# hzeller/timg

Measured on NVIDIA H100. Metric: Mpixels/s scale+dither+sixel-encode @4K→cell, higher is better.
Workload: dtype u8/f32

## Files before the change

### timg_b200/csrc/sixel.cu

```cuda
#include <cstdlib>

#include "sixel.cuh"

namespace b200timg {

constexpr int PT = 1024;

__device__ __forceinline__ int pick_plane(int d0, int d1, int d2) {
    const double lum[3] = {0.2989, 0.5866, 0.1145};
    const int spreads[3] = {d0 << 3, d1 << 3, d2 << 3};
    int plane = 0; double best = 0.0;
#pragma unroll
    for (int p = 0; p < 3; ++p) { const double sp = lum[p] * (double)spreads[p]; if (sp > best) { plane = p; best = sp; } }
    return plane;
}

template <bool SMEM_TABLES>
__global__ void __launch_bounds__(PT)
sixel_palette_kernel(const uint32_t *__restrict__ fb, int w, int h, SixelWork W) {
    extern __shared__ uint32_t s_hist[];
    __shared__ uint32_t s_w[PT / 32];
    __shared__ int b_ind[256], b_col[256], b_med[256], t_ind[256], t_col[256], t_med[256];
    __shared__ uint32_t b_sum[256], b_low[256], t_sum[256], t_low[256];
    __shared__ int s_mn[3], s_mx[3];
    __shared__ uint32_t s_cnt[32], s_base[32], s_run[32];
    __shared__ unsigned short s_wh[32][32];
    __shared__ uint32_t w_cnt[32][32], w_base[32][32], w_run[32][32];
    __shared__ int s_todo[32], s_ntodo, s_boxes, s_done;
    __shared__ unsigned long long s_med;

    const int f = blockIdx.x, tid = threadIdx.x, lane = tid & 31, wid = tid >> 5;
    const long long npix = (long long)w * h;
    const uint32_t *frame = fb + (long long)f * npix;
    SixelFrameHdr *hdr = W.hdr + f;
    const int t_words = W.ent_cap > 16384 ? W.ent_cap : 16384;
    uint32_t *E = SMEM_TABLES ? s_hist + t_words : W.ent_a + (long long)f * W.ent_cap;
    uint32_t *T = SMEM_TABLES ? s_hist : W.ent_b + (long long)f * W.ent_cap;

    unsigned long long step_px = (unsigned long long)npix / 18383ull;
    if ((unsigned long long)npix < 18383ull) step_px = 6;
    if (step_px == 0) step_px = 1;
    const long long ns = (npix + (long long)step_px - 1) / (long long)step_px;

    for (int i = tid; i < 16384; i += PT) s_hist[i] = 0;
    __syncthreads();
    for (long long k = tid; k < ns; k += PT) {
        const uint32_t b = hash15(frame[k * (long long)step_px]);
        atomicAdd(&s_hist[b >> 1], 1u << (16 * (b & 1)));
    }
    __syncthreads();
    uint32_t mine = 0;
    for (int k = 0; k < 16; ++k) { const uint32_t v = s_hist[tid * 16 + k]; mine += ((v & 0xffff) != 0) + ((v >> 16) != 0); }
    uint32_t n_ent;
    uint32_t pos = block_excl_scan<PT>(mine, s_w, n_ent);
    for (int k = 0; k < 16; ++k) {
        const uint32_t v = s_hist[tid * 16 + k];
        const uint32_t b0 = (uint32_t)(tid * 32 + 2 * k);
        if (v & 0xffff) E[pos++] = (b0 << 16) | (v & 0xffff);
        if (v >> 16) E[pos++] = ((b0 + 1) << 16) | (v >> 16);
    }
    __syncthreads();
    if (tid == 0) { hdr->origcolors = n_ent; hdr->diffuse = n_ent > 256 ? 1 : 0; }
    if (n_ent <= 256) {
        if (tid < 256) {
            uint32_t pal = 0;
            if ((uint32_t)tid < n_ent) { const uint32_t e = E[tid]; pal = (key5(e, 0) << 3) | (key5(e, 1) << 11) | (key5(e, 2) << 19); }
            hdr->palette[tid] = pal;
        }
        if (tid == 0) hdr->ncolors = n_ent;
        return;
    }
    {
        uint32_t sacc = 0;
        for (uint32_t i = tid; i < n_ent; i += PT) sacc += E[i] & 0xffff;
        uint32_t total; const uint32_t dummy = block_excl_scan<PT>(sacc, s_w, total); (void)dummy;
        if (tid == 0) { b_ind[0] = 0; b_col[0] = (int)n_ent; b_sum[0] = total; b_med[0] = -1; s_boxes = 1; s_done = 0; }
    }
    for (;;) {
        __syncthreads();
        if (wid == 0) {
            const int nb = s_boxes;
            int count = 0;
            for (int c0 = 0; c0 < nb; c0 += 32) {
                const int j = c0 + lane;
                const bool flag = j < nb && b_col[j] >= 2 && b_med[j] < 0;
                const uint32_t m = __ballot_sync(0xffffffffu, flag);
                const int pos = count + __popc(m & ((1u << lane) - 1));
                if (flag && pos < 32) s_todo[pos] = j;
                count += __popc(m);
            }
            if (lane == 0) s_ntodo = min(count, 32);
        }
        __syncthreads();
        const int ntodo = s_ntodo;
        for (int t = 0; t < ntodo; ++t) {
            const int bi = s_todo[t];
            const int start = b_ind[bi], size = b_col[bi];
            if (size <= 1024) continue;
            const uint32_t sm = b_sum[bi];
            uint32_t *B = E + start, *TB = T + start;
            if (tid == 0) { s_mn[0] = s_mn[1] = s_mn[2] = 31; s_mx[0] = s_mx[1] = s_mx[2] = 0; s_med = ~0ull; }
            if (tid < 32) { s_cnt[tid] = 0; s_run[tid] = 0; }
            __syncthreads();
            int mn0 = 31, mn1 = 31, mn2 = 31, mx0 = 0, mx1 = 0, mx2 = 0;
            for (int i = tid; i < size; i += PT) {
                const uint32_t e = B[i];
                const int k0 = key5(e, 0), k1 = key5(e, 1), k2 = key5(e, 2);
                mn0 = min(mn0, k0); mx0 = max(mx0, k0); mn1 = min(mn1, k1); mx1 = max(mx1, k1); mn2 = min(mn2, k2); mx2 = max(mx2, k2);
            }
#pragma unroll
            for (int d = 16; d; d >>= 1) {
                mn0 = min(mn0, __shfl_xor_sync(0xffffffffu, mn0, d)); mx0 = max(mx0, __shfl_xor_sync(0xffffffffu, mx0, d));
                mn1 = min(mn1, __shfl_xor_sync(0xffffffffu, mn1, d)); mx1 = max(mx1, __shfl_xor_sync(0xffffffffu, mx1, d));
                mn2 = min(mn2, __shfl_xor_sync(0xffffffffu, mn2, d)); mx2 = max(mx2, __shfl_xor_sync(0xffffffffu, mx2, d));
            }
            if (lane == 0) {
                atomicMin(&s_mn[0], mn0); atomicMax(&s_mx[0], mx0); atomicMin(&s_mn[1], mn1); atomicMax(&s_mx[1], mx1);
                atomicMin(&s_mn[2], mn2); atomicMax(&s_mx[2], mx2);
            }
            __syncthreads();
            const int plane = pick_plane(s_mx[0] - s_mn[0], s_mx[1] - s_mn[1], s_mx[2] - s_mn[2]);
            for (int i = tid; i < size; i += PT) atomicAdd(&s_cnt[key5(B[i], plane)], 1u);
            __syncthreads();
            if (tid < 32) {
                const uint32_t c = s_cnt[tid]; uint32_t inc = c;
#pragma unroll
                for (int d = 1; d < 32; d <<= 1) { const uint32_t o = __shfl_up_sync(0xffffffffu, inc, d); if (lane >= d) inc += o; }
                s_base[tid] = inc - c;
            }
            for (int t0 = 0; t0 < size; t0 += PT) {
                s_wh[wid][lane] = 0;
                __syncthreads();
                const int i = t0 + tid;
                const bool valid = i < size;
                uint32_t e = 0, k = 0, rank = 0;
                const uint32_t vmask = __ballot_sync(0xffffffffu, valid);
                if (valid) {
                    e = B[i]; k = key5(e, plane);
                    const uint32_t m = __match_any_sync(vmask, k);
                    rank = __popc(m & ((1u << lane) - 1));
                    if (rank == 0) s_wh[wid][k] = (unsigned short)__popc(m);
                }
                __syncthreads();
                if (valid) {
                    uint32_t pp = s_base[k] + s_run[k] + rank;
                    for (int w2 = 0; w2 < wid; ++w2) pp += s_wh[w2][k];
                    TB[pp] = e;
                }
                __syncthreads();
                if (tid < 32) { uint32_t acc = 0; for (int w2 = 0; w2 < 32; ++w2) acc += s_wh[w2][tid]; s_run[tid] += acc; }
                __syncthreads();
            }
            for (int i = tid; i < size; i += PT) B[i] = TB[i];
            __syncthreads();
            {
                const uint32_t half = sm / 2;
                uint32_t carry = 0;
                for (int t0 = 0; t0 < size; t0 += PT) {
                    const int i = t0 + tid;
                    const uint32_t c = i < size ? (B[i] & 0xffff) : 0;
                    uint32_t tot; const uint32_t before = carry + block_excl_scan<PT>(c, s_w, tot);
                    if (i >= 1 && i <= size - 2 && before >= half) atomicMin(&s_med, ((unsigned long long)i << 32) | before);
                    carry += tot;
                    __syncthreads();
                    if (s_med != ~0ull) break;
                }
            }
            __syncthreads();
            if (tid == 0) {
                if (s_med != ~0ull) { b_med[bi] = (int)(s_med >> 32); b_low[bi] = (uint32_t)s_med; }
                else { b_med[bi] = size - 1; b_low[bi] = sm - (B[size - 1] & 0xffff); }
            }
            __syncthreads();
        }
        if (wid < ntodo) {
            const int bi = s_todo[wid];
            const int start = b_ind[bi], size = b_col[bi];
            if (size <= 1024) {
                const uint32_t sm = b_sum[bi];
                uint32_t *B = E + start, *TB = T + start;
                uint32_t *cnt = w_cnt[wid], *base = w_base[wid], *run = w_run[wid];
                cnt[lane] = 0; run[lane] = 0;
                int mn0 = 31, mn1 = 31, mn2 = 31, mx0 = 0, mx1 = 0, mx2 = 0;
                for (int i = lane; i < size; i += 32) {
                    const uint32_t e = B[i];
                    const int k0 = key5(e, 0), k1 = key5(e, 1), k2 = key5(e, 2);
                    mn0 = min(mn0, k0); mx0 = max(mx0, k0); mn1 = min(mn1, k1); mx1 = max(mx1, k1); mn2 = min(mn2, k2); mx2 = max(mx2, k2);
                }
#pragma unroll
                for (int d = 16; d; d >>= 1) {
                    mn0 = min(mn0, __shfl_xor_sync(0xffffffffu, mn0, d)); mx0 = max(mx0, __shfl_xor_sync(0xffffffffu, mx0, d));
                    mn1 = min(mn1, __shfl_xor_sync(0xffffffffu, mn1, d)); mx1 = max(mx1, __shfl_xor_sync(0xffffffffu, mx1, d));
                    mn2 = min(mn2, __shfl_xor_sync(0xffffffffu, mn2, d)); mx2 = max(mx2, __shfl_xor_sync(0xffffffffu, mx2, d));
                }
                const int plane = pick_plane(mx0 - mn0, mx1 - mn1, mx2 - mn2);
                __syncwarp();
                for (int t0 = 0; t0 < size; t0 += 32) {
                    const int i = t0 + lane;
                    const bool valid = i < size;
                    const uint32_t vm = __ballot_sync(0xffffffffu, valid);
                    if (valid) {
                        const uint32_t k = key5(B[i], plane);
                        const uint32_t m = __match_any_sync(vm, k);
                        if ((m & ((1u << lane) - 1)) == 0) cnt[k] += __popc(m);
                    }
                    __syncwarp();
                }
                {
                    const uint32_t c = cnt[lane]; uint32_t inc = c;
#pragma unroll
                    for (int d = 1; d < 32; d <<= 1) { const uint32_t o = __shfl_up_sync(0xffffffffu, inc, d); if (lane >= d) inc += o; }
                    base[lane] = inc - c;
                }
                __syncwarp();
                for (int t0 = 0; t0 < size; t0 += 32) {
                    const int i = t0 + lane;
                    const bool valid = i < size;
                    const uint32_t vm = __ballot_sync(0xffffffffu, valid);
                    uint32_t k = 0, m = 0;
                    if (valid) {
                        const uint32_t e = B[i];
                        k = key5(e, plane);
                        m = __match_any_sync(vm, k);
                        TB[base[k] + run[k] + __popc(m & ((1u << lane) - 1))] = e;
                    }
                    __syncwarp();
                    if (valid && (m & ((1u << lane) - 1)) == 0) run[k] += __popc(m);
                    __syncwarp();
                }
                for (int i = lane; i < size; i += 32) B[i] = TB[i];
                __syncwarp();
                const uint32_t half = sm / 2;
                uint32_t carry = 0; int median = size - 1; uint32_t lower = 0; bool found = false;
                for (int t0 = 0; t0 < size && !found; t0 += 32) {
                    const int i = t0 + lane;
                    const uint32_t c = i < size ? (B[i] & 0xffff) : 0;
                    uint32_t inc = c;
#pragma unroll
                    for (int d = 1; d < 32; d <<= 1) { const uint32_t o = __shfl_up_sync(0xffffffffu, inc, d); if (lane >= d) inc += o; }
                    const uint32_t before = carry + inc - c;
                    const uint32_t hit = __ballot_sync(0xffffffffu, i >= 1 && i <= size - 2 && before >= half);
                    if (hit) {
                        const int src = __ffs(hit) - 1;
                        median = t0 + src; lower = __shfl_sync(0xffffffffu, before, src); found = true;
                    }
                    carry += __shfl_sync(0xffffffffu, inc, 31);
                }
                if (!found) lower = sm - (B[size - 1] & 0xffff);
                if (lane == 0) { b_med[bi] = median; b_low[bi] = lower; }
            }
        }
        __syncthreads();
        if (wid == 0) {
            int done = 0;
            for (;;) {
                const int nb = s_boxes;
                if (nb >= 256) { done = 1; break; }
                int first = 1 << 30;
                for (int j = lane; j < nb; j += 32) if (b_col[j] >= 2) { first = j; break; }
#pragma unroll
                for (int d = 16; d; d >>= 1) first = min(first, __shfl_xor_sync(0xffffffffu, first, d));
                if (first >= nb) { done = 1; break; }
                if (b_med[first] < 0) break;
                const int ia = first, in_ = nb, nb1 = nb + 1;
                const int start = b_ind[ia], size = b_col[ia], median = b_med[ia];
                const uint32_t sm = b_sum[ia], lower = b_low[ia];
                __syncwarp();
                if (lane == 0) {
                    b_col[ia] = median; b_sum[ia] = lower; b_med[ia] = -1;
                    b_ind[in_] = start + median; b_col[in_] = size - median; b_sum[in_] = sm - lower; b_med[in_] = -1;
                    s_boxes = nb1;
                }
                __syncwarp();
                const uint32_t sA = lower, sN = sm - lower;
                int cntA = 0, cntN = 0;
                int my_pos[8];
#pragma unroll
                for (int c = 0; c < 8; ++c) {
                    const int j = c * 32 + lane;
                    bool pa = false, pn = false;
                    my_pos[c] = -1;
                    if (j < nb1 && j != ia && j != in_) {
                        const uint32_t me = b_sum[j];
                        my_pos[c] = j - (j > ia ? 1 : 0) + (((sA > me) || (sA == me && ia < j)) ? 1 : 0) + ((sN > me) ? 1 : 0);
                        pa = (me > sA) || (me == sA && j < ia);
                        pn = me >= sN;
                    }
                    cntA += __popc(__ballot_sync(0xffffffffu, pa));
                    cntN += __popc(__ballot_sync(0xffffffffu, pn));
                }
#pragma unroll
                for (int c = 0; c < 8; ++c) {
                    const int j = c * 32 + lane;
                    if (j < nb1) {
                        int pos = my_pos[c];
                        if (j == ia) pos = cntA + (sN > sA ? 1 : 0);
                        if (j == in_) pos = cntN + (sA >= sN ? 1 : 0);
                        t_ind[pos] = b_ind[j]; t_col[pos] = b_col[j]; t_sum[pos] = b_sum[j]; t_med[pos] = b_med[j]; t_low[pos] = b_low[j];
                    }
                }
                __syncwarp();
#pragma unroll
                for (int c = 0; c < 8; ++c) {
                    const int j = c * 32 + lane;
                    if (j < nb1) { b_ind[j] = t_ind[j]; b_col[j] = t_col[j]; b_sum[j] = t_sum[j]; b_med[j] = t_med[j]; b_low[j] = t_low[j]; }
                }
                __syncwarp();
            }
            if (lane == 0) s_done = done;
        }
        __syncthreads();
        if (s_done) break;
    }
    if (tid < 256) {
        uint32_t pal = 0;
        if (tid < s_boxes) {
            uint32_t s0 = 0, s1 = 0, s2 = 0; const int st = b_ind[tid], n = b_col[tid];
            for (int i = 0; i < n; ++i) { const uint32_t e = E[st + i]; s0 += key5(e, 0) << 3; s1 += key5(e, 1) << 3; s2 += key5(e, 2) << 3; }
            pal = (s0 / (uint32_t)n) | ((s1 / (uint32_t)n) << 8) | ((s2 / (uint32_t)n) << 16);
        }
        hdr->palette[tid] = pal;
    }
    if (tid == 0) hdr->ncolors = 256;
}

__global__ void __launch_bounds__(256)
sixel_lut_kernel(SixelWork W) {
    __shared__ uint32_t s_pal[256];
    const int f = blockIdx.y;
    const SixelFrameHdr *hdr = W.hdr + f;
    s_pal[threadIdx.x] = hdr->palette[threadIdx.x];
    __syncthreads();
    const int n = (int)hdr->ncolors;
    const uint32_t cell = blockIdx.x * 256 + threadIdx.x;
    const uint32_t c = (((cell >> 10) & 31) << 3 | 4) | ((((cell >> 5) & 31) << 3 | 4) << 8) | (((cell & 31) << 3 | 4) << 16);
    uint32_t best = 0xffffffffu;
    for (int i = 0; i < n; ++i) {
        const uint32_t d = __vabsdiffu4(c, s_pal[i]);
        best = min(best, (__dp4a(d, d, 0u) << 8) | (uint32_t)i);
    }
    const uint32_t bi = n > 0 ? (best & 255u) : 0u;
    W.lut[(long long)f * 32768 + cell] = (uint8_t)bi;
}

__global__ void __launch_bounds__(256)
sixel_map_kernel(const uint32_t *__restrict__ fb, long long npix, SixelWork W) {
    const int f = blockIdx.y;
    if (W.hdr[f].diffuse) return;
    const uint8_t *lut = W.lut + (long long)f * 32768;
    const long long stride = (long long)gridDim.x * blockDim.x;
    for (long long i = (long long)blockIdx.x * blockDim.x + threadIdx.x; i < npix; i += stride)
        W.index[(long long)f * npix + i] = lut[hash15(fb[(long long)f * npix + i])];
}

constexpr uint32_t EZ = 256u | (256u << 9) | (256u << 18);
__device__ __forceinline__ int fs_tap(int v, int e, int k) {
    const int t = e * k;
    const int q = (t + ((t >> 31) & 15)) >> 4;
    return min(255, max(0, v + q));
}
struct FsErr {
    int e[3], b[3];
    __device__ __forceinline__ void zero() { e[0] = e[1] = e[2] = 0; b[0] = b[1] = b[2] = 0; }
    __device__ __forceinline__ void set(int r, int g, int bl) {
        e[0] = r; e[1] = g; e[2] = bl;
        b[0] = (r >> 31) & 15; b[1] = (g >> 31) & 15; b[2] = (bl >> 31) & 15;
    }
    __device__ __forceinline__ void unpack(uint32_t p) { set((int)(p & 511) - 256, (int)((p >> 9) & 511) - 256, (int)((p >> 18) & 511) - 256); }
    __device__ __forceinline__ uint32_t pack() const { return (uint32_t)(e[0] + 256) | ((uint32_t)(e[1] + 256) << 9) | ((uint32_t)(e[2] + 256) << 18); }
};
__device__ __forceinline__ int fs_add(int v, const FsErr &er, int c, int k) {
    return min(255, max(0, v + ((er.e[c] * k + er.b[c]) >> 4)));
}
constexpr int DW_MAX = 24;
constexpr int DCH = 16;
constexpr int DIN_STRIDE = DCH + 1;
constexpr int DOUT_STRIDE = 20;
constexpr int DWARP_SMEM = 2 * 32 * DIN_STRIDE * 4 + 32 * DOUT_STRIDE;

__global__ void __launch_bounds__(DW_MAX * 32)
sixel_dither_kernel(const uint32_t *__restrict__ fb, int w, int h, int nwarps, SixelWork W) {
    extern __shared__ __align__(16) uint8_t s_dyn[];
    __shared__ uint32_t s_pal[256];
    __shared__ volatile int s_progress[2048];
    const int f = blockIdx.x;
    const SixelFrameHdr *hdr = W.hdr + f;
    if (!hdr->diffuse) return;
    const int tid = threadIdx.x, lane = tid & 31, wid = tid >> 5;
    const int nthreads = nwarps * 32;
    uint8_t *s_lut = s_dyn;
    for (int i = tid; i < 32768 / 4; i += nthreads)
        reinterpret_cast<uint32_t *>(s_lut)[i] = reinterpret_cast<const uint32_t *>(W.lut + (long long)f * 32768)[i];
    for (int i = tid; i < 256; i += nthreads) s_pal[i] = hdr->palette[i];
    for (int i = tid; i < W.nb32; i += nthreads) s_progress[i] = 0;
    __syncthreads();
    uint32_t *s_in = reinterpret_cast<uint32_t *>(s_dyn + 32768 + (size_t)wid * DWARP_SMEM);
    uint8_t *s_out = reinterpret_cast<uint8_t *>(s_in + 2 * 32 * DIN_STRIDE);
    const uint32_t *frame = fb + (long long)f * w * h;
    uint8_t *index = W.index + (long long)f * w * h;
    uint32_t *bnd = W.boundary + (long long)f * W.nb32 * w;
    const int hrow = lane >> 4, hcol = lane & 15;

    for (int band = wid; band < W.nb32; band += nwarps) {
        const int y = band * 32 + lane;
        const bool row_ok = y < h;
        const bool last_row = (y == h - 1);
        const uint32_t *bin = band > 0 ? bnd + (long long)(band - 1) * w : nullptr;
        uint32_t *bout = bnd + (long long)band * w;
        uint32_t last_e = EZ;
        FsErr up_m1, up_0, up_p1, own, e_first;
        up_m1.zero(); up_0.zero(); up_p1.zero(); own.zero(); e_first.zero();
        const int steps = w + 62, nchunks = (steps + DCH - 1) / DCH;
        uint32_t pre[16];
        auto load_chunk = [&](int c) {
#pragma unroll
            for (int i = 0; i < 16; ++i) {
                const int r = 2 * i + hrow, yy = band * 32 + r, x = c * DCH - 2 * r + hcol;
                pre[i] = (yy < h && x >= 0 && x < w) ? frame[(long long)yy * w + x] : 0u;
            }
        };
        auto store_chunk = [&](int c) {
            uint32_t *t = s_in + (c & 1) * 32 * DIN_STRIDE;
#pragma unroll
            for (int i = 0; i < 16; ++i) t[(2 * i + hrow) * DIN_STRIDE + hcol] = pre[i];
        };
        load_chunk(0); store_chunk(0);
        __syncwarp();
        for (int c = 0; c < nchunks; ++c) {
            const int t0 = c * DCH;
            if (c + 1 < nchunks) load_chunk(c + 1);
            uint32_t binreg = EZ;
            if (band > 0) {
                const int need = min(w, t0 + DCH + 1);
                if (lane == 0) { while (s_progress[band - 1] < need) __nanosleep(32); __threadfence_block(); }
                __syncwarp();
                const int bx = t0 + 1 + lane;
                if (lane < DCH && bx < w) binreg = __ldcg(bin + bx);
                if (c == 0 && lane == 0) up_p1.unpack(__ldcg(bin));
            }
            const uint32_t *tin = s_in + (c & 1) * 32 * DIN_STRIDE + lane * DIN_STRIDE;
            uint32_t bkeep = EZ;
            const bool interior = (t0 - 62 >= 1) && (t0 + DCH - 1 <= w - 2) && (band * 32 + 31 < h - 1);
            if (interior) {
#pragma unroll 4
                for (int j = 0; j < DCH; ++j) {
                    uint32_t recv = __shfl_up_sync(0xffffffffu, last_e, 1);
                    const uint32_t b0 = __shfl_sync(0xffffffffu, binreg, j);
                    if (lane == 0) recv = b0;
                    up_m1 = up_0; up_0 = up_p1; up_p1.unpack(recv);
                    const uint32_t px = tin[j];
                    int v[3] = {(int)(px & 0xff), (int)((px >> 8) & 0xff), (int)((px >> 16) & 0xff)};
#pragma unroll
                    for (int ch = 0; ch < 3; ++ch) {
                        v[ch] = fs_add(v[ch], up_m1, ch, 1);
                        v[ch] = fs_add(v[ch], up_0, ch, 5);
                        v[ch] = fs_add(v[ch], up_p1, ch, 3);
                        v[ch] = fs_add(v[ch], own, ch, 7);
                    }
                    const uint32_t cell = ((uint32_t)(v[0] >> 3) << 10) | ((uint32_t)(v[1] >> 3) << 5) | (uint32_t)(v[2] >> 3);
                    const uint32_t ci = s_lut[cell];
                    const uint32_t pal = s_pal[ci];
                    own.set(v[0] - (int)(pal & 0xff), v[1] - (int)((pal >> 8) & 0xff), v[2] - (int)((pal >> 16) & 0xff));
                    last_e = own.pack();
                    s_out[lane * DOUT_STRIDE + j] = (uint8_t)ci;
                    const uint32_t e31 = __shfl_sync(0xffffffffu, last_e, 31);
                    if (lane == j) bkeep = e31;
                }
            } else {
#pragma unroll 2
                for (int j = 0; j < DCH; ++j) {
                    const int t = t0 + j, x = t - 2 * lane;
                    uint32_t recv = __shfl_up_sync(0xffffffffu, last_e, 1);
                    const uint32_t b0 = __shfl_sync(0xffffffffu, binreg, j);
                    if (lane == 0) recv = b0;
                    up_m1 = up_0; up_0 = up_p1; up_p1.unpack(recv);
                    uint32_t ci = 0;
                    if (x >= 0 && x < w && row_ok) {
                        const uint32_t px = tin[j];
                        int v[3] = {(int)(px & 0xff), (int)((px >> 8) & 0xff), (int)((px >> 16) & 0xff)};
#pragma unroll
                        for (int ch = 0; ch < 3; ++ch) {
                            v[ch] = fs_add(v[ch], up_m1, ch, 1);
                            v[ch] = fs_add(v[ch], up_0, ch, 5);
                            v[ch] = fs_add(v[ch], up_p1, ch, 3);
                            if (x == w - 1) v[ch] = fs_add(v[ch], e_first, ch, 3);
                            v[ch] = fs_add(v[ch], own, ch, 7);
                        }
                        const uint32_t cell = ((uint32_t)(v[0] >> 3) << 10) | ((uint32_t)(v[1] >> 3) << 5) | (uint32_t)(v[2] >> 3);
                        ci = s_lut[cell];
                        const uint32_t pal = s_pal[ci];
                        if (x < w - 1 && !last_row) own.set(v[0] - (int)(pal & 0xff), v[1] - (int)((pal >> 8) & 0xff), v[2] - (int)((pal >> 16) & 0xff));
                        else own.zero();
                        if (x == 0) e_first = own;
                        last_e = own.pack();
                    } else if (x >= w) {
                        last_e = EZ;
                    }
                    s_out[lane * DOUT_STRIDE + j] = (uint8_t)ci;
                    const uint32_t e31 = __shfl_sync(0xffffffffu, last_e, 31);
                    if (lane == j) bkeep = e31;
                }
            }
            __syncwarp();
#pragma unroll
            for (int i = 0; i < 16; ++i) {
                const int r = 2 * i + hrow, yy = band * 32 + r, x = t0 - 2 * r + hcol;
                if (yy < h && x >= 0 && x < w) index[(long long)yy * w + x] = s_out[r * DOUT_STRIDE + hcol];
            }
            {
                const int x = t0 + lane - 62;
                if (lane < DCH && x >= 0 && x < w) __stcg(bout + x, bkeep);
                __threadfence_block();
                __syncwarp();
                const int done = min(w, t0 + DCH - 62);
                if (lane == 0 && done > 0) s_progress[band] = done;
            }
            if (c + 1 < nchunks) store_chunk(c + 1);
            __syncwarp();
        }
    }
}

__device__ __forceinline__ uint32_t ndig4(uint32_t v) { return 1u + (v >= 10u) + (v >= 100u) + (v >= 1000u); }
__device__ __forceinline__ char *put_num4(char *o, uint32_t v) {
    const uint32_t d3 = v / 1000u, r3 = v - d3 * 1000u, d2 = r3 / 100u, r2 = r3 - d2 * 100u, d1 = r2 / 10u, d0 = r2 - d1 * 10u;
    if (v >= 1000u) *o++ = (char)('0' + d3);
    if (v >= 100u) *o++ = (char)('0' + d2);
    if (v >= 10u) *o++ = (char)('0' + d1);
    *o++ = (char)('0' + d0);
    return o;
}
__device__ __forceinline__ uint32_t rle_len(uint32_t n) { return n > 3u ? 2u + ndig4(n) : n; }
__device__ __forceinline__ char *put_rle(char *o, uint32_t n, char ch) {
    if (n > 3u) { *o++ = '!'; o = put_num4(o, n); *o++ = ch; }
    else { if (n > 0u) *o++ = ch; if (n > 1u) *o++ = ch; if (n > 2u) *o++ = ch; }
    return o;
}

constexpr int ET = 512, EW = ET / 32;
__device__ __forceinline__ uint32_t ent_pack(uint32_t c, uint32_t x, uint32_t bits) { return (c << 18) | (x << 6) | bits; }

struct EmitGeom { int w, h, cols_per_warp; };

template <typename F>
__device__ __forceinline__ void walk_runs(const uint32_t *sorted, int lo, int hi, int n, F emit) {
    int i = lo;
    uint32_t prev = 0; bool have_prev = false;
    if (i > 0 && i < hi) { prev = sorted[i - 1]; have_prev = true; }
    while (i < hi) {
        const uint32_t e = sorted[i];
        if (have_prev && e == prev + 64u) { prev = e; ++i; continue; }
        uint32_t cur = e, L = 1;
        while (i + (int)L < n && sorted[i + L] == cur + 64u) { cur += 64u; ++L; }
        const uint32_t c = e >> 18, x = (e >> 6) & 4095u;
        const bool same_colour = have_prev && (prev >> 18) == c;
        emit(c, e & 63u, same_colour ? x - ((prev >> 6) & 4095u) - 1u : x, L, !same_colour);
        prev = cur; have_prev = true;
        i += (int)L;
    }
}

__global__ void __launch_bounds__(ET)
sixel_emit_kernel(EmitGeom G, SixelWork W) {
    extern __shared__ uint32_t s_sorted[];
    __shared__ uint32_t s_cnt[EW][256];
    __shared__ uint32_t s_mask[EW * 256];
    __shared__ uint32_t s_w[ET / 32];
    const int band = blockIdx.x, f = blockIdx.y, tid = threadIdx.x, lane = tid & 31, wid = tid >> 5;
    const int w = G.w;
    const SixelFrameHdr *hdr = W.hdr + f;
    const uint8_t *idx = W.index + ((long long)f * G.h + (long long)band * 6) * w;

    for (int i = tid; i < EW * 256; i += ET) { (&s_cnt[0][0])[i] = 0; s_mask[i] = 0; }
    __syncthreads();

    const int x_lo = wid * G.cols_per_warp, x_hi = min(w, x_lo + G.cols_per_warp);
    uint32_t *cnt = s_cnt[wid];
    for (int x = x_lo + lane; x < x_hi; x += 32) {
        uint32_t col[6], bits[6];
        const uint32_t valid = column_entries(idx, w, x, col, bits);
#pragma unroll
        for (int s = 0; s < 6; ++s) if (valid & (1u << s)) atomicAdd(&cnt[col[s]], 1u);
    }
    __syncthreads();
    uint32_t tot_c = 0;
    if (tid < 256) for (int k = 0; k < EW; ++k) tot_c += s_cnt[k][tid];
    uint32_t n_ent; const uint32_t cb = block_excl_scan<ET>(tid < 256 ? tot_c : 0, s_w, n_ent);
    if (tid < 256) {
        uint32_t run = cb;
        for (int k = 0; k < EW; ++k) { const uint32_t v = s_cnt[k][tid]; s_cnt[k][tid] = run; run += v; }
    }
    __syncthreads();
    uint32_t *M = s_mask + wid * 256;
    const uint32_t lt = (1u << lane) - 1;
    for (int x0 = x_lo; x0 < x_hi; x0 += 32) {
        const int x = x0 + lane;
        uint32_t col[6], bits[6];
        const uint32_t valid = x < x_hi ? column_entries(idx, w, x, col, bits) : 0u;
#pragma unroll
        for (int s = 0; s < 6; ++s) if (valid & (1u << s)) atomicOr(&M[col[s]], 1u << lane);
        __syncwarp();
        uint32_t mk[6];
#pragma unroll
        for (int s = 0; s < 6; ++s)
            if (valid & (1u << s)) {
                mk[s] = M[col[s]];
                s_sorted[cnt[col[s]] + __popc(mk[s] & lt)] = ent_pack(col[s], (uint32_t)x, bits[s]);
            }
        __syncwarp();
#pragma unroll
        for (int s = 0; s < 6; ++s)
            if ((valid & (1u << s)) && (mk[s] & lt) == 0) { cnt[col[s]] += (uint32_t)__popc(mk[s]); M[col[s]] = 0; }
        __syncwarp();
    }
    __syncthreads();
    const int n = (int)n_ent;
    const uint32_t minc = s_sorted[0] >> 18;
    const int per = (n + ET - 1) / ET, lo = min(n, tid * per), hi = min(n, lo + per);
    uint32_t local = 0;
    walk_runs(s_sorted, lo, hi, n, [&](uint32_t c, uint32_t, uint32_t gap, uint32_t len, bool first) {
        local += rle_len(gap) + rle_len(len) + (first ? 1u + ndig4(c) + (c != minc ? 1u : 0u) : 0u);
    });
    uint32_t band_total; uint32_t at = block_excl_scan<ET>(local, s_w, band_total);
    if (tid == 0) W.band_bytes[(long long)f * W.nbands + band] = band_total;
    char *o = W.scratch + ((size_t)f * W.nbands + band) * W.band_cap + at;
    walk_runs(s_sorted, lo, hi, n, [&](uint32_t c, uint32_t bits, uint32_t gap, uint32_t len, bool first) {
        if (first) { if (c != minc) *o++ = '$'; *o++ = '#'; o = put_num4(o, c); }
        o = put_rle(o, gap, '?');
        o = put_rle(o, len, (char)('?' + bits));
    });
}

constexpr int SLOT_WORDS = 22;
constexpr int STASH_STEPS = 6;
constexpr uint32_t SLOT_MAX = 4 * (SLOT_WORDS - 3);
static_assert(SLOT_WORDS * ET >= 2 * EW * 256, "the slots alias the sort's tables");

struct DecTable { uint32_t v[4096]; };
constexpr DecTable make_dec_table() {
    DecTable t{};
    for (uint32_t n = 0; n < 4096; ++n) {
        uint32_t s = 0, m = n, nd = 0;
        do { s = (s << 8) | (0x30u + m % 10u); m /= 10u; ++nd; } while (m);
        t.v[n] = s;
    }
    return t;
}
__device__ const DecTable k_dec = make_dec_table();
__device__ __forceinline__ uint32_t dec4(uint32_t v, uint32_t &nd) {
    const uint32_t s = __ldg(&k_dec.v[v]);
    nd = 4u - ((uint32_t)__clz((int)s) >> 3);
    return s;
}
__device__ __forceinline__ unsigned long long rle_piece4(uint32_t n, uint32_t ch, uint32_t &len) {
    if (n > 3u) {
        uint32_t nd;
        const uint32_t d = dec4(n, nd);
        len = 2u + nd;
        return 0x21ull | ((unsigned long long)d << 8) | ((unsigned long long)ch << (8u * (1u + nd)));
    }
    len = n;
    return (unsigned long long)((ch * 0x010101u) & ((1u << (8u * n)) - 1u));
}
__device__ __forceinline__ void slot_append(uint32_t *slot, uint32_t &pos, uint32_t &cur, unsigned long long v, uint32_t len) {
    const uint32_t sh = 8u * (pos & 3u);
    const uint32_t lo = (uint32_t)v, hi = (uint32_t)(v >> 32);
    const uint32_t w0 = cur | (lo << sh);
    const uint32_t w1 = __funnelshift_l(lo, hi, sh);
    const uint32_t w2 = sh ? (hi >> (32u - sh)) : 0u;
    uint32_t *p = slot + min(pos >> 2, (uint32_t)(SLOT_WORDS - 3)) * ET;
    p[0] = w0; p[ET] = w1; p[2 * ET] = w2;
    const uint32_t np = pos + len, adv = (np >> 2) - (pos >> 2);
    cur = adv == 0u ? w0 : (adv == 1u ? w1 : w2);
    pos = np;
}

__global__ void __launch_bounds__(ET, 2)
sixel_emit1b_kernel(EmitGeom G, SixelWork W) {
    extern __shared__ uint32_t s_sorted[];
    __shared__ uint32_t s_tab[SLOT_WORDS * ET];
    __shared__ uint32_t s_w[ET / 32];
    const int band = blockIdx.x, f = blockIdx.y, tid = threadIdx.x, lane = tid & 31, wid = tid >> 5;
    const int w = G.w;
    const uint8_t *idx = W.index + ((long long)f * G.h + (long long)band * 6) * w;

    for (int i = tid; i < 2 * EW * 256; i += ET) s_tab[i] = 0;
    __syncthreads();
    const int x_lo = wid * G.cols_per_warp, x_hi = min(w, x_lo + G.cols_per_warp);
    uint32_t *cnt = s_tab + wid * 256, *M = s_tab + EW * 256 + wid * 256;
    const bool stash = G.cols_per_warp <= 32 * STASH_STEPS;
    uint32_t k0[STASH_STEPS], k1[STASH_STEPS], k2[STASH_STEPS];
    if (stash) {
#pragma unroll
        for (int t = 0; t < STASH_STEPS; ++t) {
            const int x = x_lo + 32 * t + lane;
            k0[t] = k1[t] = k2[t] = 0;
            if (x < x_hi) {
                uint32_t col[6], bits[6];
                const uint32_t valid = column_entries(idx, w, x, col, bits);
#pragma unroll
                for (int s = 0; s < 6; ++s) if (valid & (1u << s)) atomicAdd(&cnt[col[s]], 1u);
                k0[t] = col[0] | (col[1] << 8) | (col[2] << 16) | (col[3] << 24);
                k1[t] = col[4] | (col[5] << 8) | (valid << 16) | (bits[5] << 22);
                k2[t] = bits[0] | (bits[1] << 6) | (bits[2] << 12) | (bits[3] << 18) | (bits[4] << 24);
            }
        }
    } else {
        for (int x = x_lo + lane; x < x_hi; x += 32) {
            uint32_t col[6], bits[6];
            const uint32_t valid = column_entries(idx, w, x, col, bits);
#pragma unroll
            for (int s = 0; s < 6; ++s) if (valid & (1u << s)) atomicAdd(&cnt[col[s]], 1u);
        }
    }
    __syncthreads();
    uint32_t tot_c = 0;
    if (tid < 256) for (int k = 0; k < EW; ++k) tot_c += s_tab[k * 256 + tid];
    uint32_t n_ent; const uint32_t cb = block_excl_scan<ET>(tid < 256 ? tot_c : 0, s_w, n_ent);
    if (tid < 256) {
        uint32_t run = cb;
        for (int k = 0; k < EW; ++k) { const uint32_t v = s_tab[k * 256 + tid]; s_tab[k * 256 + tid] = run; run += v; }
    }
    __syncthreads();
    const uint32_t lt = (1u << lane) - 1;
    auto scatter_step = [&](int x, uint32_t valid, const uint32_t *col, const uint32_t *bits) {
#pragma unroll
        for (int s = 0; s < 6; ++s) if (valid & (1u << s)) atomicOr(&M[col[s]], 1u << lane);
        __syncwarp();
        uint32_t mk[6];
#pragma unroll
        for (int s = 0; s < 6; ++s)
            if (valid & (1u << s)) {
                mk[s] = M[col[s]];
                s_sorted[cnt[col[s]] + __popc(mk[s] & lt)] = ent_pack(col[s], (uint32_t)x, bits[s]);
            }
        __syncwarp();
#pragma unroll
        for (int s = 0; s < 6; ++s)
            if ((valid & (1u << s)) && (mk[s] & lt) == 0) { cnt[col[s]] += (uint32_t)__popc(mk[s]); M[col[s]] = 0; }
        __syncwarp();
    };
    if (stash) {
#pragma unroll
        for (int t = 0; t < STASH_STEPS; ++t) {
            if (x_lo + 32 * t < x_hi) {
                const uint32_t col[6] = {k0[t] & 255u, (k0[t] >> 8) & 255u, (k0[t] >> 16) & 255u, k0[t] >> 24, k1[t] & 255u, (k1[t] >> 8) & 255u};
                const uint32_t bits[6] = {k2[t] & 63u, (k2[t] >> 6) & 63u, (k2[t] >> 12) & 63u, (k2[t] >> 18) & 63u, (k2[t] >> 24) & 63u, (k1[t] >> 22) & 63u};
                scatter_step(x_lo + 32 * t + lane, (k1[t] >> 16) & 63u, col, bits);
            }
        }
    } else {
        for (int x0 = x_lo; x0 < x_hi; x0 += 32) {
            const int x = x0 + lane;
            uint32_t col[6], bits[6];
            const uint32_t valid = x < x_hi ? column_entries(idx, w, x, col, bits) : 0u;
            scatter_step(x, valid, col, bits);
        }
    }
    __syncthreads();
    const int n = (int)n_ent;
    const uint32_t minc = s_sorted[0] >> 18;
    const int per = (n + ET - 1) / ET, lo = min(n, tid * per), hi = min(n, lo + per);
    uint32_t *slot = s_tab + tid;
    uint32_t pos = 0, cur = 0;
    bool ovf = false;
    walk_runs(s_sorted, lo, hi, n, [&](uint32_t c, uint32_t bits, uint32_t gap, uint32_t len, bool first) {
        uint32_t pl;
        if (first) {
            uint32_t nd;
            unsigned long long v = 0x23ull | ((unsigned long long)dec4(c, nd) << 8);
            pl = 1u + nd;
            if (c != minc) { v = 0x24ull | (v << 8); ++pl; }
            ovf |= pos > SLOT_MAX;
            slot_append(slot, pos, cur, v, pl);
        }
        uint32_t rl;
        const unsigned long long gv = rle_piece4(gap, 0x3fu, pl), rv = rle_piece4(len, 0x3fu + bits, rl);
        ovf |= pos > SLOT_MAX;
        if (pl + rl <= 8u) {
            slot_append(slot, pos, cur, gv | (rv << (8u * pl)), pl + rl);
        } else {
            slot_append(slot, pos, cur, gv, pl);
            ovf |= pos > SLOT_MAX;
            slot_append(slot, pos, cur, rv, rl);
        }
    });
    const uint32_t local = pos;
    uint32_t band_total; const uint32_t at = block_excl_scan<ET>(local, s_w, band_total);
    if (tid == 0) W.band_bytes[(long long)f * W.nbands + band] = band_total;
    char *o = W.scratch + ((size_t)f * W.nbands + band) * W.band_cap + at;
    if (!ovf) {
        const uint32_t head = min(local, (4u - (at & 3u)) & 3u);
        const uint32_t w0 = slot[0];
        for (uint32_t k = 0; k < head; ++k) o[k] = (char)(w0 >> (8u * k));
        const uint32_t nw = (local - head) >> 2;
        uint32_t *dw = reinterpret_cast<uint32_t *>(o + head);
        uint32_t a = w0;
        for (uint32_t j = 0; j < nw; ++j) {
            const uint32_t b = slot[(j + 1) * ET];
            dw[j] = __funnelshift_r(a, b, 8u * head);
            a = b;
        }
        const uint32_t done = head + 4u * nw;
        for (uint32_t k = done; k < local; ++k) o[k] = (char)(slot[(k >> 2) * ET] >> (8u * (k & 3u)));
    } else {
        walk_runs(s_sorted, lo, hi, n, [&](uint32_t c, uint32_t bits, uint32_t gap, uint32_t len, bool first) {
            if (first) { if (c != minc) *o++ = '$'; *o++ = '#'; o = put_num4(o, c); }
            o = put_rle(o, gap, '?');
            o = put_rle(o, len, (char)('?' + bits));
        });
    }
}

__global__ void __launch_bounds__(256)
sixel_layout_kernel(int w, int h, SixelWork W) {
    __shared__ uint32_t s_w[8];
    __shared__ uint32_t s_carry;
    const int f = blockIdx.x, tid = threadIdx.x;
    SixelFrameHdr *hdr = W.hdr + f;
    uint32_t len = 0;
    if ((uint32_t)tid < hdr->ncolors) {
        const uint32_t p = hdr->palette[tid];
        const uint32_t r = ((p & 0xff) * 100 + 127) / 255, g = (((p >> 8) & 0xff) * 100 + 127) / 255, b = (((p >> 16) & 0xff) * 100 + 127) / 255;
        len = 1 + ndig_u((uint32_t)tid) + 3 + ndig_u(r) + 1 + ndig_u(g) + 1 + ndig_u(b);
    }
    uint32_t pal_total; (void)block_excl_scan<256>(len, s_w, pal_total);
    const uint32_t header = 8 + ndig_u((uint32_t)w) + 1 + ndig_u((uint32_t)h) + pal_total;
    if (tid == 0) s_carry = header;
    __syncthreads();
    uint32_t *bb = W.band_bytes + (long long)f * W.nbands;
    for (int b0 = 0; b0 < W.nbands; b0 += 256) {
        const int b = b0 + tid;
        const uint32_t v = b < W.nbands ? bb[b] + (b > 0 ? 1u : 0u) : 0;
        uint32_t tot; const uint32_t at = block_excl_scan<256>(v, s_w, tot);
        if (b < W.nbands) W.band_off[(long long)f * W.nbands + b] = s_carry + at + (b > 0 ? 1u : 0u);
        __syncthreads();
        if (tid == 0) s_carry += tot;
        __syncthreads();
    }
    if (tid == 0) { hdr->header_len = header; hdr->frame_size = s_carry + 2; }
}

__global__ void __launch_bounds__(1024)
sixel_sizes_to_offsets_kernel(const SixelFrameHdr *__restrict__ hdr, int n, uint64_t *__restrict__ offsets) {
    __shared__ unsigned long long s_wv[32];
    __shared__ unsigned long long c_run;
    const int tid = threadIdx.x, lane = tid & 31, wid = tid >> 5;
    if (tid == 0) c_run = 0;
    __syncthreads();
    for (int i0 = 0; i0 < n; i0 += 1024) {
        const int i = i0 + tid;
        unsigned long long v = i < n ? hdr[i].frame_size : 0ull;
        const unsigned long long mine = v;
#pragma unroll
        for (int d = 1; d < 32; d <<= 1) { const unsigned long long o = __shfl_up_sync(0xffffffffu, v, d); if (lane >= d) v += o; }
        if (lane == 31) s_wv[wid] = v;
        __syncthreads();
        unsigned long long pre = 0, tot = 0;
        for (int k = 0; k < 32; ++k) { if (k < wid) pre += s_wv[k]; tot += s_wv[k]; }
        if (i < n) offsets[i] = c_run + pre + v - mine;
        __syncthreads();
        if (tid == 0) c_run += tot;
        __syncthreads();
    }
    if (tid == 0) offsets[n] = c_run;
}

__global__ void __launch_bounds__(256)
sixel_compact_kernel(int w, int h, SixelWork W, const uint64_t *__restrict__ offsets, char *__restrict__ out,
                     unsigned long long out_cap) {
    __shared__ uint32_t s_w[8];
    const int band = blockIdx.x, f = blockIdx.y, tid = threadIdx.x;
    const SixelFrameHdr *hdr = W.hdr + f;
    const unsigned long long fbase = offsets[f];
    if (fbase + hdr->frame_size > out_cap) return;
    const uint32_t boff = W.band_off[(long long)f * W.nbands + band];
    const uint32_t n = W.band_bytes[(long long)f * W.nbands + band];
    const char *src = W.scratch + ((size_t)f * W.nbands + band) * W.band_cap;
    char *dst = out + fbase + boff;
    {
        const uint32_t head = min(n, (uint32_t)((4 - (reinterpret_cast<uintptr_t>(dst) & 3)) & 3));
        if ((uint32_t)tid < head) dst[tid] = src[tid];
        const uint32_t nw = (n - head) >> 2, m = head & 3;
        const uint32_t *sw = reinterpret_cast<const uint32_t *>(src + head - m);
        uint32_t *dw = reinterpret_cast<uint32_t *>(dst + head);
        for (uint32_t j = tid; j < nw; j += 256) dw[j] = m ? __funnelshift_r(sw[j], sw[j + 1], 8 * m) : sw[j];
        const uint32_t done = head + (nw << 2);
        if (done + tid < n) dst[done + tid] = src[done + tid];
    }
    if (tid == 0) {
        if (band > 0) dst[-1] = '-';
        if (band == W.nbands - 1) { out[fbase + hdr->frame_size - 2] = '\033'; out[fbase + hdr->frame_size - 1] = '\\'; }
    }
    if (band == 0) {
        if (tid == 0) {
            char *o = out + fbase;
            *o++ = '\033'; *o++ = 'P'; *o++ = 'q'; *o++ = '"'; *o++ = '1'; *o++ = ';'; *o++ = '1'; *o++ = ';';
            o = put_num_u(o, (uint32_t)w); *o++ = ';'; o = put_num_u(o, (uint32_t)h);
        }
        const uint32_t fixed = 8 + ndig_u((uint32_t)w) + 1 + ndig_u((uint32_t)h);
        uint32_t len = 0, r = 0, g = 0, b = 0;
        if ((uint32_t)tid < hdr->ncolors) {
            const uint32_t p = hdr->palette[tid];
            r = ((p & 0xff) * 100 + 127) / 255; g = (((p >> 8) & 0xff) * 100 + 127) / 255; b = (((p >> 16) & 0xff) * 100 + 127) / 255;
            len = 1 + ndig_u((uint32_t)tid) + 3 + ndig_u(r) + 1 + ndig_u(g) + 1 + ndig_u(b);
        }
        uint32_t tot; const uint32_t at = block_excl_scan<256>(len, s_w, tot);
        if (len) {
            char *q = out + fbase + fixed + at;
            *q++ = '#'; q = put_num_u(q, (uint32_t)tid); *q++ = ';'; *q++ = '2'; *q++ = ';';
            q = put_num_u(q, r); *q++ = ';'; q = put_num_u(q, g); *q++ = ';'; q = put_num_u(q, b);
        }
    }
}

static size_t align_up(size_t v, size_t a) { return (v + a - 1) / a * a; }

struct SixelPlan {
    SixelWork W;
    bool emit_v1, dither_v1;
    int emit_mode;
    EmitGeom G;
    size_t emit_smem, o_d2_bnd, o_d2_prog;
    long long npix;
};

static int sixel_plan(b200timg_ctx *ctx, int w, int h, int n_frames, bool reserve, SixelPlan *S) {
    if (h % 6) return ctx->fail(B200TIMG_EINVAL, "sixel: height %d is not a multiple of 6", h);
    if (n_frames > 65535) return ctx->fail(B200TIMG_EINVAL, "sixel: too many frames for one launch");
    SixelWork &W = S->W;
    const long long npix = (long long)w * h;
    S->npix = npix;
    long long step_px = npix / 18383; if (npix < 18383) step_px = 6; if (step_px == 0) step_px = 1;
    const long long ns = (npix + step_px - 1) / step_px;
    W.ent_cap = (int)std::min<long long>(32768, ns);
    W.nb32 = (h + 31) / 32; W.nbands = h / 6;
    if (W.nb32 > 2048) return ctx->fail(B200TIMG_EINVAL, "sixel: frame too tall");
    size_t off = 0;
    const size_t o_hdr = off; off += align_up(sizeof(SixelFrameHdr) * n_frames, 256);
    const size_t o_ea = off; off += align_up(sizeof(uint32_t) * (size_t)W.ent_cap * n_frames, 256);
    const size_t o_eb = off; off += align_up(sizeof(uint32_t) * (size_t)W.ent_cap * n_frames, 256);
    const size_t o_lut = off; off += align_up((size_t)32768 * n_frames, 256);
    const size_t o_idx = off; off += align_up((size_t)npix * n_frames, 256);
    const size_t o_bnd = off; off += align_up(sizeof(uint32_t) * (size_t)W.nb32 * w * n_frames, 256);
    const size_t o_bb = off; off += align_up(sizeof(uint32_t) * (size_t)W.nbands * n_frames, 256);
    const size_t o_bo = off; off += align_up(sizeof(uint32_t) * (size_t)W.nbands * n_frames, 256);
    W.band_cap = align_up((size_t)w * 42 + 256 * 5 + 16, 256);
    const size_t o_scr = off;
    {
        const bool v1_fits = w <= 4095 && sizeof(uint32_t) * (size_t)6 * w <= (size_t)(227 - 36) * 1024;
        const bool v1b_fits = w <= 4095 && sizeof(uint32_t) * (size_t)6 * w <= (size_t)(227 - 47) * 1024;
        int mode = v1b_fits ? 4 : v1_fits ? 1 : 2;
        if (getenv("B200TIMG_EMIT_V2")) mode = 2;
        if (const char *e = getenv("B200TIMG_EMIT")) mode = atoi(e);
        if (mode < 1 || mode > 4 || (mode == 1 && !v1_fits) || (mode == 4 && !v1b_fits)) mode = 2;
        S->emit_mode = mode;
        S->emit_v1 = mode == 1 || mode == 4;
    }
    if (S->emit_v1) off += W.band_cap * W.nbands * n_frames;
    S->dither_v1 = getenv("B200TIMG_DITHER_V1") != nullptr;
    size_t d_bnd, d_prog;
    const size_t o_d2 = off; off += sixel_dither_workspace(w, h, n_frames, &d_bnd, &d_prog);
    size_t e_hdr, e_desc, e_ctl;
    const size_t o_e2 = off; off += sixel_emit_workspace(w, h, n_frames, &e_hdr, &e_desc, &e_ctl);
    if (reserve) B2_CUDA(ctx, ctx->sixel_work.reserve(off));
    if (!ctx->sixel_work.p || ctx->sixel_work.cap < off) return ctx->fail(B200TIMG_EINVAL, "sixel: write phase without prepare");
    ctx->sixel_idx_off = o_idx;
    char *base = ctx->sixel_work.as<char>();
    W.hdr = reinterpret_cast<SixelFrameHdr *>(base + o_hdr);
    W.ent_a = reinterpret_cast<uint32_t *>(base + o_ea); W.ent_b = reinterpret_cast<uint32_t *>(base + o_eb);
    W.lut = reinterpret_cast<uint8_t *>(base + o_lut); W.index = reinterpret_cast<uint8_t *>(base + o_idx);
    W.boundary = reinterpret_cast<uint32_t *>(base + o_bnd); W.band_bytes = reinterpret_cast<uint32_t *>(base + o_bb);
    W.band_off = reinterpret_cast<uint32_t *>(base + o_bo); W.scratch = base + o_scr;
    W.hdr_bytes = base + o_e2 + e_hdr;
    W.desc = reinterpret_cast<unsigned long long *>(base + o_e2 + e_desc);
    W.ctl = reinterpret_cast<uint32_t *>(base + o_e2 + e_ctl);
    S->o_d2_bnd = o_d2 + d_bnd; S->o_d2_prog = o_d2 + d_prog;
    S->G.w = w; S->G.h = h; S->G.cols_per_warp = ((w + EW - 1) / EW + 31) / 32 * 32;
    const size_t smem_limit = 227 * 1024 - 36 * 1024;
    S->emit_smem = sizeof(uint32_t) * (size_t)6 * w;
    if (!ctx->sixel_attrs_set) {
        B2_CUDA(ctx, cudaFuncSetAttribute(sixel_palette_kernel<false>, cudaFuncAttributeMaxDynamicSharedMemorySize, 65536));
        B2_CUDA(ctx, cudaFuncSetAttribute(sixel_emit_kernel, cudaFuncAttributeMaxDynamicSharedMemorySize, (int)smem_limit));
        B2_CUDA(ctx, cudaFuncSetAttribute(sixel_emit1b_kernel, cudaFuncAttributeMaxDynamicSharedMemorySize, (227 - 47) * 1024));
        B2_CUDA(ctx, cudaFuncSetAttribute(sixel_dither_kernel, cudaFuncAttributeMaxDynamicSharedMemorySize, 32768 + DW_MAX * DWARP_SMEM));
        B2_CUDA(ctx, cudaFuncSetAttribute(sixel_palette_kernel<true>, cudaFuncAttributeMaxDynamicSharedMemorySize, 200 * 1024));
        ctx->sixel_attrs_set = true;
    }
    return B200TIMG_OK;
}

int launch_sixel_front(b200timg_ctx *ctx, const uint8_t *d_fb, int w, int h, int n_total, int f0, int n, bool reserve) {
    if ((reinterpret_cast<uintptr_t>(d_fb) & 3)) return ctx->fail(B200TIMG_EINVAL, "sixel: framebuffer must be 4-byte aligned");
    SixelPlan S;
    B2_TRY(sixel_plan(ctx, w, h, n_total, reserve, &S));
    SixelWork W = S.W;
    const long long npix = S.npix;
    W.hdr += f0; W.ent_a += (long long)f0 * W.ent_cap; W.ent_b += (long long)f0 * W.ent_cap; W.lut += (long long)f0 * 32768;
    W.index += (long long)f0 * npix; W.boundary += (long long)f0 * W.nb32 * w;
    W.band_bytes += (long long)f0 * W.nbands; W.band_off += (long long)f0 * W.nbands;
    W.scratch += (size_t)f0 * W.nbands * W.band_cap;
    const uint32_t *fb = reinterpret_cast<const uint32_t *>(d_fb) + (long long)f0 * npix;
    char *base = ctx->sixel_work.as<char>();
    B2_KERNEL(ctx, "sixel_palette_kernel");
    {
        const size_t t_words = W.ent_cap > 16384 ? (size_t)W.ent_cap : 16384;
        const size_t smem_tables = sizeof(uint32_t) * (t_words + (size_t)W.ent_cap);
        if (smem_tables <= 200 * 1024) sixel_palette_kernel<true><<<n, PT, smem_tables, ctx->stream>>>(fb, w, h, W);
        else sixel_palette_kernel<false><<<n, PT, 65536, ctx->stream>>>(fb, w, h, W);
    }
    B2_LAUNCH_CHECK(ctx);
    B2_KERNEL(ctx, "sixel_lut_kernel");
    sixel_lut_kernel<<<dim3(128, n), 256, 0, ctx->stream>>>(W);
    B2_LAUNCH_CHECK(ctx);
    {
        long long blocks = (npix + 255) / 256; if (blocks > 64) blocks = 64;
        B2_KERNEL(ctx, "sixel_map_kernel");
        sixel_map_kernel<<<dim3((unsigned)blocks, n), 256, 0, ctx->stream>>>(fb, npix, W);
        B2_LAUNCH_CHECK(ctx);
    }
    if (!S.dither_v1) {
        B2_TRY(launch_sixel_dither(ctx, fb, w, h, n, n_total, W, base + S.o_d2_bnd + sizeof(uint4) * (size_t)f0 * W.nb32 * w,
                                   base + S.o_d2_prog + sizeof(int) * (size_t)f0 * W.nb32));
    } else {
        B2_KERNEL(ctx, "sixel_dither_kernel");
        const int rounds = (W.nb32 + DW_MAX - 1) / DW_MAX;
        const int nwarps = (W.nb32 + rounds - 1) / rounds;
        const size_t dsmem = 32768 + (size_t)nwarps * DWARP_SMEM;
        sixel_dither_kernel<<<n, nwarps * 32, dsmem, ctx->stream>>>(fb, w, h, nwarps, W);
        B2_LAUNCH_CHECK(ctx);
    }
    if (S.emit_v1) {
        B2_KERNEL(ctx, "sixel_emit_kernel");
        if (S.emit_mode == 4) sixel_emit1b_kernel<<<dim3(W.nbands, n), ET, S.emit_smem, ctx->stream>>>(S.G, W);
        else sixel_emit_kernel<<<dim3(W.nbands, n), ET, S.emit_smem, ctx->stream>>>(S.G, W);
        B2_LAUNCH_CHECK(ctx);
    }
    return B200TIMG_OK;
}

int launch_sixel_back(b200timg_ctx *ctx, int w, int h, int n_frames, char *d_out, size_t out_cap, uint64_t *d_offsets, int phases) {
    SixelPlan S;
    B2_TRY(sixel_plan(ctx, w, h, n_frames, false, &S));
    const SixelWork &W = S.W;
    if (!S.emit_v1) {
        if (!(phases & 2)) return B200TIMG_OK;
        if (S.emit_mode == 2) return launch_sixel_emit(ctx, w, h, n_frames, W, d_out, out_cap, d_offsets);
        return launch_sixel_emit3(ctx, w, h, n_frames, W, d_out, out_cap, d_offsets);
    }
    if (phases & 1) {
        B2_KERNEL(ctx, "sixel_layout_kernel");
        sixel_layout_kernel<<<n_frames, 256, 0, ctx->stream>>>(w, h, W);
        B2_LAUNCH_CHECK(ctx);
        B2_KERNEL(ctx, "sixel_sizes_to_offsets_kernel");
        sixel_sizes_to_offsets_kernel<<<1, 1024, 0, ctx->stream>>>(W.hdr, n_frames, d_offsets);
        B2_LAUNCH_CHECK(ctx);
    }
    if (!(phases & 2)) return B200TIMG_OK;
    B2_KERNEL(ctx, "sixel_compact_kernel");
    sixel_compact_kernel<<<dim3(W.nbands, n_frames), 256, 0, ctx->stream>>>(w, h, W, d_offsets, d_out, (unsigned long long)out_cap);
    B2_LAUNCH_CHECK(ctx);
    return B200TIMG_OK;
}

int launch_sixel(b200timg_ctx *ctx, const uint8_t *d_fb, int w, int h, int n_frames, char *d_out,
                 size_t out_cap, uint64_t *d_offsets, int phases) {
    if (phases & 1) B2_TRY(launch_sixel_front(ctx, d_fb, w, h, n_frames, 0, n_frames, true));
    return launch_sixel_back(ctx, w, h, n_frames, d_out, out_cap, d_offsets, phases);
}

int sixel_debug_fetch(b200timg_ctx *ctx, uint32_t *h_palette, uint32_t *h_counts, uint8_t *h_index, size_t index_bytes) {
    if (!ctx->sixel_work.p) return ctx->fail(B200TIMG_EINVAL, "sixel: nothing encoded yet");
    SixelFrameHdr host;
    B2_CUDA(ctx, cudaMemcpyAsync(&host, ctx->sixel_work.p, sizeof host, cudaMemcpyDeviceToHost, ctx->stream));
    if (h_index && index_bytes)
        B2_CUDA(ctx, cudaMemcpyAsync(h_index, ctx->sixel_work.as<char>() + ctx->sixel_idx_off, index_bytes,
                                     cudaMemcpyDeviceToHost, ctx->stream));
    B2_CUDA(ctx, cudaStreamSynchronize(ctx->stream));
    if (h_palette) memcpy(h_palette, host.palette, sizeof host.palette);
    if (h_counts) { h_counts[0] = host.ncolors; h_counts[1] = host.origcolors; }
    return B200TIMG_OK;
}

}
```

### timg_b200/csrc/sixel.cuh

```cuda
#pragma once
#include "common.cuh"

namespace b200timg {

constexpr int SIXEL_HDR_CAP = 4672;

struct SixelFrameHdr {
    uint32_t ncolors, origcolors, diffuse, header_len;
    uint32_t frame_size, pad0, pad1, pad2;
    uint32_t palette[256];
};

struct SixelWork {
    SixelFrameHdr *hdr;
    uint32_t *ent_a, *ent_b;
    uint8_t *lut;
    uint8_t *index;
    uint32_t *boundary;
    uint32_t *band_bytes;
    uint32_t *band_off;
    char *scratch;
    size_t band_cap;
    int ent_cap, nb32, nbands;
    char *hdr_bytes;
    unsigned long long *desc;
    uint32_t *ctl;
};

__device__ __forceinline__ uint32_t hash15(uint32_t px) {
    return ((px & 0xf8) << 7) | ((px >> 6) & 0x3e0) | ((px >> 19) & 0x1f);
}
__device__ __forceinline__ uint32_t key5(uint32_t entry, int plane) { return (entry >> (26 - 5 * plane)) & 31; }

template <int NT>
__device__ __forceinline__ uint32_t block_excl_scan(uint32_t v, uint32_t *s_w , uint32_t &total) {
    const int lane = threadIdx.x & 31, wid = threadIdx.x >> 5;
    uint32_t inc = v;
#pragma unroll
    for (int d = 1; d < 32; d <<= 1) { const uint32_t o = __shfl_up_sync(0xffffffffu, inc, d); if (lane >= d) inc += o; }
    if (lane == 31) s_w[wid] = inc;
    __syncthreads();
    uint32_t pre = 0, tot = 0;
    for (int k = 0; k < NT / 32; ++k) { if (k < wid) pre += s_w[k]; tot += s_w[k]; }
    total = tot;
    __syncthreads();
    return pre + inc - v;
}


__device__ __forceinline__ uint32_t ndig_u(uint32_t v) { uint32_t n = 1; while (v >= 10) { v /= 10; ++n; } return n; }
__device__ __forceinline__ char *put_num_u(char *o, uint32_t v) {
    char tmp[10]; int n = 0;
    do { tmp[n++] = (char)('0' + v % 10); v /= 10; } while (v);
    while (n) *o++ = tmp[--n];
    return o;
}

__device__ __forceinline__ uint32_t column_entries(const uint8_t *__restrict__ idx, int w, int x, uint32_t *c, uint32_t *bits) {
#pragma unroll
    for (int i = 0; i < 6; ++i) c[i] = idx[(long long)i * w + x];
    uint32_t valid = 0;
#pragma unroll
    for (int i = 0; i < 6; ++i) {
        bool seen = false;
        uint32_t b = 0;
#pragma unroll
        for (int j = 0; j < 6; ++j) {
            if (j < i && c[j] == c[i]) seen = true;
            if (j >= i && c[j] == c[i]) b |= 1u << j;
        }
        bits[i] = b;
        if (!seen) valid |= 1u << i;
    }
    return valid;
}

int launch_sixel_emit(b200timg_ctx *ctx, int w, int h, int n_frames, const SixelWork &W, char *d_out, size_t out_cap,
                      uint64_t *d_offsets);
int launch_sixel_emit3(b200timg_ctx *ctx, int w, int h, int n_frames, const SixelWork &W, char *d_out, size_t out_cap,
                       uint64_t *d_offsets);
size_t sixel_dither_workspace(int w, int h, int n_frames, size_t *o_bnd, size_t *o_prog);
int launch_sixel_dither(b200timg_ctx *ctx, const uint32_t *fb, int w, int h, int n_frames, int n_total, const SixelWork &W, void *d_bnd, void *d_prog);
size_t sixel_emit_workspace(int w, int h, int n_frames, size_t *o_hdr_bytes, size_t *o_desc, size_t *o_ctl);

}
```

### timg_b200/csrc/sixel_dither.cu

```cuda
#include <algorithm>
#include <cstdlib>

#include "sixel.cuh"

namespace b200timg {

#ifdef CUSIM
__device__ __forceinline__ uint32_t prmt(uint32_t a, uint32_t b, uint32_t s) { return __byte_perm(a, b, s); }
#else
__device__ __forceinline__ uint32_t prmt(uint32_t a, uint32_t b, uint32_t s) {
    uint32_t d;
    asm("prmt.b32 %0, %1, %2, %3;" : "=r"(d) : "r"(a), "r"(b), "r"(s));
    return d;
}
#endif

constexpr int D2_WMAX = 24;
constexpr int D2_CH = 16;
constexpr int D2_IN_STRIDE = D2_CH + 1;
constexpr int D2_OUT_STRIDE = 20;
constexpr int D2_WARP_SMEM = 2 * 32 * D2_IN_STRIDE * 4 + 32 * D2_OUT_STRIDE + D2_CH * 16;

struct TapW { uint32_t r, g, b; };

template <int K> __device__ __forceinline__ uint32_t tap_rg(const TapW &t) {
    constexpr uint32_t sel = (uint32_t)K | ((8u | K) << 4) | ((4u + K) << 8) | ((8u | (4u + K)) << 12);
    return prmt(t.r, t.g, sel);
}
template <int K> __device__ __forceinline__ uint32_t tap_b(const TapW &t) {
    constexpr uint32_t sel = (uint32_t)K | ((8u | K) << 4) | (4u << 8) | (4u << 12);
    return prmt(t.b, 0u, sel);
}
__device__ __forceinline__ uint32_t add_clamp(uint32_t v, uint32_t t) { return __viaddmin_s16x2_relu(v, t, 0x00ff00ffu); }

struct Dither2Geom { int w, h, nb32, bands_per_cta, nwarps; unsigned spin_ns; };

__global__ void __launch_bounds__(D2_WMAX * 32)
sixel_dither2_kernel(const uint32_t *__restrict__ fb, Dither2Geom G, SixelWork W, uint4 *__restrict__ bnd_all, int *__restrict__ gprog_all) {
    extern __shared__ __align__(16) uint8_t s_dyn2[];
    __shared__ uint2 s_pal2[256];
    __shared__ uint32_t s_tap[512];
    __shared__ volatile int s_progress[2048];
    const int f = blockIdx.y, g = blockIdx.x;
    const SixelFrameHdr *hdr = W.hdr + f;
    if (!hdr->diffuse) return;
    const int tid = threadIdx.x, lane = tid & 31, wid = tid >> 5;
    const int nthreads = G.nwarps * 32, w = G.w, h = G.h;
    uint8_t *s_lut = s_dyn2;
    for (int i = tid; i < 32768 / 16; i += nthreads)
        reinterpret_cast<uint4 *>(s_lut)[i] = reinterpret_cast<const uint4 *>(W.lut + (long long)f * 32768)[i];
    for (int i = tid; i < 256; i += nthreads) {
        const uint32_t p = hdr->palette[i];
        s_pal2[i] = make_uint2((256u - (p & 0xff)) | ((256u - ((p >> 8) & 0xff)) << 16), (256u - ((p >> 16) & 0xff)) | (256u << 16));
    }
    for (int i = tid; i < 512; i += nthreads) {
        const int e = i - 256;
        const int t7 = e * 7 / 16, t3 = e * 3 / 16, t5 = e * 5 / 16, t1 = e / 16;
        s_tap[i] = (uint32_t)(t7 & 0xff) | ((uint32_t)(t3 & 0xff) << 8) | ((uint32_t)(t5 & 0xff) << 16) | ((uint32_t)(t1 & 0xff) << 24);
    }
    const int band_lo = g * G.bands_per_cta, band_hi = min(G.nb32, band_lo + G.bands_per_cta);
    const int nlocal = band_hi - band_lo;
    for (int i = tid; i < nlocal; i += nthreads) s_progress[i] = 0;
    __syncthreads();
    uint32_t *s_in = reinterpret_cast<uint32_t *>(s_dyn2 + 32768 + (size_t)wid * D2_WARP_SMEM);
    uint8_t *s_out = reinterpret_cast<uint8_t *>(s_in + 2 * 32 * D2_IN_STRIDE);
    uint4 *s_bnd = reinterpret_cast<uint4 *>(s_out + 32 * D2_OUT_STRIDE);
    const uint32_t *frame = fb + (long long)f * w * h;
    uint8_t *index = W.index + (long long)f * w * h;
    uint4 *bnd = bnd_all + (long long)f * G.nb32 * w;
    volatile int *gprog = gprog_all + (long long)f * G.nb32;
    const int hrow = lane >> 4, hcol = lane & 15;
    const int qrow = lane >> 3, qcol = lane & 7;
    const bool even_w = (w & 1) == 0;
    const TapW Z = {0u, 0u, 0u};

    for (int band = band_lo + wid; band < band_hi; band += G.nwarps) {
        const int lb = band - band_lo;
        const int y = band * 32 + lane;
        const bool row_ok = y < h, last_row = (y == h - 1);
        const bool prev_remote = band > 0 && lb == 0;
        const bool publish_remote = band + 1 < G.nb32 && band + 1 == band_hi;
        const uint4 *bin = band > 0 ? bnd + (long long)(band - 1) * w : nullptr;
        uint4 *bout = bnd + (long long)band * w;
        TapW own = Z, a0 = Z, a1 = Z, a2 = Z, e_first = Z;
        const int steps = w + 62, nchunks = (steps + D2_CH - 1) / D2_CH;
        uint32_t pre[16];
        auto load_chunk = [&](int c) {
            if (even_w) {
#pragma unroll
                for (int i = 0; i < 8; ++i) {
                    const int r = 4 * i + qrow, yy = band * 32 + r, x = c * D2_CH - 2 * r + 2 * qcol;
                    uint2 v = make_uint2(0u, 0u);
                    if (yy < h && x >= 0 && x < w) v = *reinterpret_cast<const uint2 *>(frame + (long long)yy * w + x);
                    pre[2 * i] = v.x; pre[2 * i + 1] = v.y;
                }
            } else {
#pragma unroll
                for (int i = 0; i < 16; ++i) {
                    const int r = 2 * i + hrow, yy = band * 32 + r, x = c * D2_CH - 2 * r + hcol;
                    pre[i] = (yy < h && x >= 0 && x < w) ? frame[(long long)yy * w + x] : 0u;
                }
            }
        };
        auto store_chunk = [&](int c) {
            uint32_t *t = s_in + (c & 1) * 32 * D2_IN_STRIDE;
            if (even_w) {
#pragma unroll
                for (int i = 0; i < 8; ++i) {
                    uint32_t *q = t + (4 * i + qrow) * D2_IN_STRIDE + 2 * qcol;
                    q[0] = pre[2 * i]; q[1] = pre[2 * i + 1];
                }
            } else {
#pragma unroll
                for (int i = 0; i < 16; ++i) t[(2 * i + hrow) * D2_IN_STRIDE + hcol] = pre[i];
            }
        };
        load_chunk(0); store_chunk(0);
        __syncwarp();
        for (int c = 0; c < nchunks; ++c) {
            const int t0 = c * D2_CH;
            if (c + 1 < nchunks) load_chunk(c + 1);
            if (band > 0) {
                const int need = min(w, t0 + D2_CH + 1);
                if (lane == 0) {
                    if (prev_remote) { while (gprog[band - 1] < need) __nanosleep(G.spin_ns); __threadfence(); }
                    else { while (s_progress[lb - 1] < need) __nanosleep(G.spin_ns); __threadfence_block(); }
                }
                __syncwarp();
                const int bx = t0 + 1 + lane;
                if (lane < D2_CH) s_bnd[lane] = bx < w ? __ldcg(bin + bx) : make_uint4(0u, 0u, 0u, 0u);
                if (c == 0 && lane == 0) { const uint4 q = __ldcg(bin); a0.r = q.x; a0.g = q.y; a0.b = q.z; }
                __syncwarp();
            }
            const uint32_t *tin = s_in + (c & 1) * 32 * D2_IN_STRIDE + lane * D2_IN_STRIDE;
            const bool interior = (t0 - 62 >= 1) && (t0 + D2_CH - 1 <= w - 2) && (band * 32 + 31 < h - 1);
            if (interior) {
#pragma unroll 4
                for (int j = 0; j < D2_CH; ++j) {
                    TapW n;
                    n.r = __shfl_up_sync(0xffffffffu, own.r, 1); n.g = __shfl_up_sync(0xffffffffu, own.g, 1); n.b = __shfl_up_sync(0xffffffffu, own.b, 1);
                    if (lane == 0) { if (band > 0) { const uint4 q = s_bnd[j]; n.r = q.x; n.g = q.y; n.b = q.z; } else n = Z; }
                    a2 = a1; a1 = a0; a0 = n;
                    const uint32_t px = tin[j];
                    uint32_t vrg = prmt(px, 0u, 0x4140u), vb = prmt(px, 0u, 0x4442u);
                    vrg = add_clamp(vrg, tap_rg<3>(a2)); vb = add_clamp(vb, tap_b<3>(a2));
                    vrg = add_clamp(vrg, tap_rg<2>(a1)); vb = add_clamp(vb, tap_b<2>(a1));
                    vrg = add_clamp(vrg, tap_rg<1>(a0)); vb = add_clamp(vb, tap_b<1>(a0));
                    vrg = add_clamp(vrg, tap_rg<0>(own)); vb = add_clamp(vb, tap_b<0>(own));
                    const uint32_t cell = ((vrg & 0xf8u) << 7) | ((vrg >> 14) & 0x3e0u) | (vb >> 3);
                    const uint32_t ci = s_lut[cell];
                    const uint2 np = s_pal2[ci];
                    const uint32_t erg = vrg + np.x, eb = vb + np.y;
                    own.r = s_tap[erg & 0x1ffu]; own.g = s_tap[erg >> 16]; own.b = s_tap[eb & 0x1ffu];
                    s_out[lane * D2_OUT_STRIDE + j] = (uint8_t)ci;
                    if (lane == 31) __stcg(bout + (t0 + j - 62), make_uint4(own.r, own.g, own.b, 0u));
                }
            } else {
#pragma unroll 2
                for (int j = 0; j < D2_CH; ++j) {
                    const int t = t0 + j, x = t - 2 * lane;
                    TapW n;
                    n.r = __shfl_up_sync(0xffffffffu, own.r, 1); n.g = __shfl_up_sync(0xffffffffu, own.g, 1); n.b = __shfl_up_sync(0xffffffffu, own.b, 1);
                    if (lane == 0) { if (band > 0) { const uint4 q = s_bnd[j]; n.r = q.x; n.g = q.y; n.b = q.z; } else n = Z; }
                    a2 = a1; a1 = a0; a0 = n;
                    uint32_t ci = 0;
                    if (x >= 0 && x < w && row_ok) {
                        const uint32_t px = tin[j];
                        uint32_t vrg = prmt(px, 0u, 0x4140u), vb = prmt(px, 0u, 0x4442u);
                        vrg = add_clamp(vrg, tap_rg<3>(a2)); vb = add_clamp(vb, tap_b<3>(a2));
                        vrg = add_clamp(vrg, tap_rg<2>(a1)); vb = add_clamp(vb, tap_b<2>(a1));
                        vrg = add_clamp(vrg, tap_rg<1>(a0)); vb = add_clamp(vb, tap_b<1>(a0));
                        if (x == w - 1) { vrg = add_clamp(vrg, tap_rg<1>(e_first)); vb = add_clamp(vb, tap_b<1>(e_first)); }
                        vrg = add_clamp(vrg, tap_rg<0>(own)); vb = add_clamp(vb, tap_b<0>(own));
                        const uint32_t cell = ((vrg & 0xf8u) << 7) | ((vrg >> 14) & 0x3e0u) | (vb >> 3);
                        ci = s_lut[cell];
                        if (x < w - 1 && !last_row) {
                            const uint2 np = s_pal2[ci];
                            const uint32_t erg = vrg + np.x, eb = vb + np.y;
                            own.r = s_tap[erg & 0x1ffu]; own.g = s_tap[erg >> 16]; own.b = s_tap[eb & 0x1ffu];
                        } else {
                            own = Z;
                        }
                        if (x == 0) e_first = own;
                        if (lane == 31) __stcg(bout + x, make_uint4(own.r, own.g, own.b, 0u));
                    } else if (x >= w) {
                        own = Z;
                    }
                    s_out[lane * D2_OUT_STRIDE + j] = (uint8_t)ci;
                }
            }
            __syncwarp();
            if (even_w) {
#pragma unroll
                for (int i = 0; i < 8; ++i) {
                    const int r = 4 * i + qrow, yy = band * 32 + r, x = t0 - 2 * r + 2 * qcol;
                    if (yy < h && x >= 0 && x < w)
                        *reinterpret_cast<unsigned short *>(index + (long long)yy * w + x) =
                            *reinterpret_cast<const unsigned short *>(s_out + r * D2_OUT_STRIDE + 2 * qcol);
                }
            } else {
#pragma unroll
                for (int i = 0; i < 16; ++i) {
                    const int r = 2 * i + hrow, yy = band * 32 + r, x = t0 - 2 * r + hcol;
                    if (yy < h && x >= 0 && x < w) index[(long long)yy * w + x] = s_out[r * D2_OUT_STRIDE + hcol];
                }
            }
            {
                const int done = min(w, t0 + D2_CH - 62);
                if (lane == 31 && done > 0) {
                    if (publish_remote) { __threadfence(); gprog[band] = done; }
                    __threadfence_block();
                    s_progress[lb] = done;
                }
            }
            if (c + 1 < nchunks) store_chunk(c + 1);
            __syncwarp();
        }
    }
}

size_t sixel_dither_workspace(int w, int h, int n_frames, size_t *o_bnd, size_t *o_prog) {
    const size_t nb32 = (size_t)(h + 31) / 32;
    size_t off = 0;
    *o_bnd = off; off += (sizeof(uint4) * nb32 * (size_t)w * n_frames + 255) / 256 * 256;
    *o_prog = off; off += (sizeof(int) * nb32 * n_frames + 255) / 256 * 256;
    return off;
}

int launch_sixel_dither(b200timg_ctx *ctx, const uint32_t *fb, int w, int h, int n_frames, int n_total, const SixelWork &W, void *d_bnd, void *d_prog) {
    Dither2Geom G;
    G.w = w; G.h = h; G.nb32 = (h + 31) / 32;
    G.spin_ns = 256;
    if (const char *e = getenv("B200TIMG_DITHER_SPIN")) G.spin_ns = (unsigned)std::max(0, std::min(atoi(e), 100000));
    int per_frame = 1;
    if (n_total < ctx->sm_count) {
        per_frame = std::max(1, std::min(ctx->sm_count / n_total, (G.nb32 + 7) / 8));
        if (const char *e = getenv("B200TIMG_DITHER_SPLIT")) per_frame = std::max(1, std::min(atoi(e), G.nb32));
        if ((long long)per_frame * n_frames > ctx->sm_count) per_frame = std::max(1, ctx->sm_count / n_frames);
    }
    G.bands_per_cta = (G.nb32 + per_frame - 1) / per_frame;
    per_frame = (G.nb32 + G.bands_per_cta - 1) / G.bands_per_cta;
    int wmax = D2_WMAX;
    if (const char *e = getenv("B200TIMG_DITHER_WARPS")) wmax = std::max(1, std::min(atoi(e), D2_WMAX));
    const int rounds = (G.bands_per_cta + wmax - 1) / wmax;
    G.nwarps = (G.bands_per_cta + rounds - 1) / rounds;
    if (G.bands_per_cta > 2048) return ctx->fail(B200TIMG_EINVAL, "sixel: frame too tall");
    const size_t smem = 32768 + (size_t)G.nwarps * D2_WARP_SMEM;
    B2_CUDA(ctx, cudaFuncSetAttribute(sixel_dither2_kernel, cudaFuncAttributeMaxDynamicSharedMemorySize, 32768 + D2_WMAX * D2_WARP_SMEM));
    if (per_frame > 1) B2_CUDA(ctx, cudaMemsetAsync(d_prog, 0, sizeof(int) * (size_t)G.nb32 * n_frames, ctx->stream));
    B2_KERNEL(ctx, "sixel_dither2_kernel");
    sixel_dither2_kernel<<<dim3(per_frame, n_frames), G.nwarps * 32, smem, ctx->stream>>>(fb, G, W, static_cast<uint4 *>(d_bnd), static_cast<int *>(d_prog));
    B2_LAUNCH_CHECK(ctx);
    return B200TIMG_OK;
}

}
```

Before: 70270.

## Overhaul dither2 with cp.async prefetch, batched boundary publish, and drop legacy dither kernel

```diff
diff --git a/timg_b200/csrc/sixel.cu b/timg_b200/csrc/sixel.cu
--- a/timg_b200/csrc/sixel.cu
+++ b/timg_b200/csrc/sixel.cu
@@ -351,174 +351,6 @@
     const long long stride = (long long)gridDim.x * blockDim.x;
     for (long long i = (long long)blockIdx.x * blockDim.x + threadIdx.x; i < npix; i += stride)
         W.index[(long long)f * npix + i] = lut[hash15(fb[(long long)f * npix + i])];
-}
-
-constexpr uint32_t EZ = 256u | (256u << 9) | (256u << 18);
-__device__ __forceinline__ int fs_tap(int v, int e, int k) {
-    const int t = e * k;
-    const int q = (t + ((t >> 31) & 15)) >> 4;
-    return min(255, max(0, v + q));
-}
-struct FsErr {
-    int e[3], b[3];
-    __device__ __forceinline__ void zero() { e[0] = e[1] = e[2] = 0; b[0] = b[1] = b[2] = 0; }
-    __device__ __forceinline__ void set(int r, int g, int bl) {
-        e[0] = r; e[1] = g; e[2] = bl;
-        b[0] = (r >> 31) & 15; b[1] = (g >> 31) & 15; b[2] = (bl >> 31) & 15;
-    }
-    __device__ __forceinline__ void unpack(uint32_t p) { set((int)(p & 511) - 256, (int)((p >> 9) & 511) - 256, (int)((p >> 18) & 511) - 256); }
-    __device__ __forceinline__ uint32_t pack() const { return (uint32_t)(e[0] + 256) | ((uint32_t)(e[1] + 256) << 9) | ((uint32_t)(e[2] + 256) << 18); }
-};
-__device__ __forceinline__ int fs_add(int v, const FsErr &er, int c, int k) {
-    return min(255, max(0, v + ((er.e[c] * k + er.b[c]) >> 4)));
-}
-constexpr int DW_MAX = 24;
-constexpr int DCH = 16;
-constexpr int DIN_STRIDE = DCH + 1;
-constexpr int DOUT_STRIDE = 20;
-constexpr int DWARP_SMEM = 2 * 32 * DIN_STRIDE * 4 + 32 * DOUT_STRIDE;
-
-__global__ void __launch_bounds__(DW_MAX * 32)
-sixel_dither_kernel(const uint32_t *__restrict__ fb, int w, int h, int nwarps, SixelWork W) {
-    extern __shared__ __align__(16) uint8_t s_dyn[];
-    __shared__ uint32_t s_pal[256];
-    __shared__ volatile int s_progress[2048];
-    const int f = blockIdx.x;
-    const SixelFrameHdr *hdr = W.hdr + f;
-    if (!hdr->diffuse) return;
-    const int tid = threadIdx.x, lane = tid & 31, wid = tid >> 5;
-    const int nthreads = nwarps * 32;
-    uint8_t *s_lut = s_dyn;
-    for (int i = tid; i < 32768 / 4; i += nthreads)
-        reinterpret_cast<uint32_t *>(s_lut)[i] = reinterpret_cast<const uint32_t *>(W.lut + (long long)f * 32768)[i];
-    for (int i = tid; i < 256; i += nthreads) s_pal[i] = hdr->palette[i];
-    for (int i = tid; i < W.nb32; i += nthreads) s_progress[i] = 0;
-    __syncthreads();
-    uint32_t *s_in = reinterpret_cast<uint32_t *>(s_dyn + 32768 + (size_t)wid * DWARP_SMEM);
-    uint8_t *s_out = reinterpret_cast<uint8_t *>(s_in + 2 * 32 * DIN_STRIDE);
-    const uint32_t *frame = fb + (long long)f * w * h;
-    uint8_t *index = W.index + (long long)f * w * h;
-    uint32_t *bnd = W.boundary + (long long)f * W.nb32 * w;
-    const int hrow = lane >> 4, hcol = lane & 15;
-
-    for (int band = wid; band < W.nb32; band += nwarps) {
-        const int y = band * 32 + lane;
-        const bool row_ok = y < h;
-        const bool last_row = (y == h - 1);
-        const uint32_t *bin = band > 0 ? bnd + (long long)(band - 1) * w : nullptr;
-        uint32_t *bout = bnd + (long long)band * w;
-        uint32_t last_e = EZ;
-        FsErr up_m1, up_0, up_p1, own, e_first;
-        up_m1.zero(); up_0.zero(); up_p1.zero(); own.zero(); e_first.zero();
-        const int steps = w + 62, nchunks = (steps + DCH - 1) / DCH;
-        uint32_t pre[16];
-        auto load_chunk = [&](int c) {
-#pragma unroll
-            for (int i = 0; i < 16; ++i) {
-                const int r = 2 * i + hrow, yy = band * 32 + r, x = c * DCH - 2 * r + hcol;
-                pre[i] = (yy < h && x >= 0 && x < w) ? frame[(long long)yy * w + x] : 0u;
-            }
-        };
-        auto store_chunk = [&](int c) {
-            uint32_t *t = s_in + (c & 1) * 32 * DIN_STRIDE;
-#pragma unroll
-            for (int i = 0; i < 16; ++i) t[(2 * i + hrow) * DIN_STRIDE + hcol] = pre[i];
-        };
-        load_chunk(0); store_chunk(0);
-        __syncwarp();
-        for (int c = 0; c < nchunks; ++c) {
-            const int t0 = c * DCH;
-            if (c + 1 < nchunks) load_chunk(c + 1);
-            uint32_t binreg = EZ;
-            if (band > 0) {
-                const int need = min(w, t0 + DCH + 1);
-                if (lane == 0) { while (s_progress[band - 1] < need) __nanosleep(32); __threadfence_block(); }
-                __syncwarp();
-                const int bx = t0 + 1 + lane;
-                if (lane < DCH && bx < w) binreg = __ldcg(bin + bx);
-                if (c == 0 && lane == 0) up_p1.unpack(__ldcg(bin));
-            }
-            const uint32_t *tin = s_in + (c & 1) * 32 * DIN_STRIDE + lane * DIN_STRIDE;
-            uint32_t bkeep = EZ;
-            const bool interior = (t0 - 62 >= 1) && (t0 + DCH - 1 <= w - 2) && (band * 32 + 31 < h - 1);
-            if (interior) {
-#pragma unroll 4
-                for (int j = 0; j < DCH; ++j) {
-                    uint32_t recv = __shfl_up_sync(0xffffffffu, last_e, 1);
-                    const uint32_t b0 = __shfl_sync(0xffffffffu, binreg, j);
-                    if (lane == 0) recv = b0;
-                    up_m1 = up_0; up_0 = up_p1; up_p1.unpack(recv);
-                    const uint32_t px = tin[j];
-                    int v[3] = {(int)(px & 0xff), (int)((px >> 8) & 0xff), (int)((px >> 16) & 0xff)};
-#pragma unroll
-                    for (int ch = 0; ch < 3; ++ch) {
-                        v[ch] = fs_add(v[ch], up_m1, ch, 1);
-                        v[ch] = fs_add(v[ch], up_0, ch, 5);
-                        v[ch] = fs_add(v[ch], up_p1, ch, 3);
-                        v[ch] = fs_add(v[ch], own, ch, 7);
-                    }
-                    const uint32_t cell = ((uint32_t)(v[0] >> 3) << 10) | ((uint32_t)(v[1] >> 3) << 5) | (uint32_t)(v[2] >> 3);
-                    const uint32_t ci = s_lut[cell];
-                    const uint32_t pal = s_pal[ci];
-                    own.set(v[0] - (int)(pal & 0xff), v[1] - (int)((pal >> 8) & 0xff), v[2] - (int)((pal >> 16) & 0xff));
-                    last_e = own.pack();
-                    s_out[lane * DOUT_STRIDE + j] = (uint8_t)ci;
-                    const uint32_t e31 = __shfl_sync(0xffffffffu, last_e, 31);
-                    if (lane == j) bkeep = e31;
-                }
-            } else {
-#pragma unroll 2
-                for (int j = 0; j < DCH; ++j) {
-                    const int t = t0 + j, x = t - 2 * lane;
-                    uint32_t recv = __shfl_up_sync(0xffffffffu, last_e, 1);
-                    const uint32_t b0 = __shfl_sync(0xffffffffu, binreg, j);
-                    if (lane == 0) recv = b0;
-                    up_m1 = up_0; up_0 = up_p1; up_p1.unpack(recv);
-                    uint32_t ci = 0;
-                    if (x >= 0 && x < w && row_ok) {
-                        const uint32_t px = tin[j];
-                        int v[3] = {(int)(px & 0xff), (int)((px >> 8) & 0xff), (int)((px >> 16) & 0xff)};
-#pragma unroll
-                        for (int ch = 0; ch < 3; ++ch) {
-                            v[ch] = fs_add(v[ch], up_m1, ch, 1);
-                            v[ch] = fs_add(v[ch], up_0, ch, 5);
-                            v[ch] = fs_add(v[ch], up_p1, ch, 3);
-                            if (x == w - 1) v[ch] = fs_add(v[ch], e_first, ch, 3);
-                            v[ch] = fs_add(v[ch], own, ch, 7);
-                        }
-                        const uint32_t cell = ((uint32_t)(v[0] >> 3) << 10) | ((uint32_t)(v[1] >> 3) << 5) | (uint32_t)(v[2] >> 3);
-                        ci = s_lut[cell];
-                        const uint32_t pal = s_pal[ci];
-                        if (x < w - 1 && !last_row) own.set(v[0] - (int)(pal & 0xff), v[1] - (int)((pal >> 8) & 0xff), v[2] - (int)((pal >> 16) & 0xff));
-                        else own.zero();
-                        if (x == 0) e_first = own;
-                        last_e = own.pack();
-                    } else if (x >= w) {
-                        last_e = EZ;
-                    }
-                    s_out[lane * DOUT_STRIDE + j] = (uint8_t)ci;
-                    const uint32_t e31 = __shfl_sync(0xffffffffu, last_e, 31);
-                    if (lane == j) bkeep = e31;
-                }
-            }
-            __syncwarp();
-#pragma unroll
-            for (int i = 0; i < 16; ++i) {
-                const int r = 2 * i + hrow, yy = band * 32 + r, x = t0 - 2 * r + hcol;
-                if (yy < h && x >= 0 && x < w) index[(long long)yy * w + x] = s_out[r * DOUT_STRIDE + hcol];
-            }
-            {
-                const int x = t0 + lane - 62;
-                if (lane < DCH && x >= 0 && x < w) __stcg(bout + x, bkeep);
-                __threadfence_block();
-                __syncwarp();
-                const int done = min(w, t0 + DCH - 62);
-                if (lane == 0 && done > 0) s_progress[band] = done;
-            }
-            if (c + 1 < nchunks) store_chunk(c + 1);
-            __syncwarp();
-        }
-    }
 }
 
 __device__ __forceinline__ uint32_t ndig4(uint32_t v) { return 1u + (v >= 10u) + (v >= 100u) + (v >= 1000u); }
@@ -918,7 +750,7 @@
 
 struct SixelPlan {
     SixelWork W;
-    bool emit_v1, dither_v1;
+    bool emit_v1;
     int emit_mode;
     EmitGeom G;
     size_t emit_smem, o_d2_bnd, o_d2_prog;
@@ -942,7 +774,6 @@
     const size_t o_eb = off; off += align_up(sizeof(uint32_t) * (size_t)W.ent_cap * n_frames, 256);
     const size_t o_lut = off; off += align_up((size_t)32768 * n_frames, 256);
     const size_t o_idx = off; off += align_up((size_t)npix * n_frames, 256);
-    const size_t o_bnd = off; off += align_up(sizeof(uint32_t) * (size_t)W.nb32 * w * n_frames, 256);
     const size_t o_bb = off; off += align_up(sizeof(uint32_t) * (size_t)W.nbands * n_frames, 256);
     const size_t o_bo = off; off += align_up(sizeof(uint32_t) * (size_t)W.nbands * n_frames, 256);
     W.band_cap = align_up((size_t)w * 42 + 256 * 5 + 16, 256);
@@ -958,7 +789,6 @@
         S->emit_v1 = mode == 1 || mode == 4;
     }
     if (S->emit_v1) off += W.band_cap * W.nbands * n_frames;
-    S->dither_v1 = getenv("B200TIMG_DITHER_V1") != nullptr;
     size_t d_bnd, d_prog;
     const size_t o_d2 = off; off += sixel_dither_workspace(w, h, n_frames, &d_bnd, &d_prog);
     size_t e_hdr, e_desc, e_ctl;
@@ -970,7 +800,7 @@
     W.hdr = reinterpret_cast<SixelFrameHdr *>(base + o_hdr);
     W.ent_a = reinterpret_cast<uint32_t *>(base + o_ea); W.ent_b = reinterpret_cast<uint32_t *>(base + o_eb);
     W.lut = reinterpret_cast<uint8_t *>(base + o_lut); W.index = reinterpret_cast<uint8_t *>(base + o_idx);
-    W.boundary = reinterpret_cast<uint32_t *>(base + o_bnd); W.band_bytes = reinterpret_cast<uint32_t *>(base + o_bb);
+    W.band_bytes = reinterpret_cast<uint32_t *>(base + o_bb);
     W.band_off = reinterpret_cast<uint32_t *>(base + o_bo); W.scratch = base + o_scr;
     W.hdr_bytes = base + o_e2 + e_hdr;
     W.desc = reinterpret_cast<unsigned long long *>(base + o_e2 + e_desc);
@@ -983,7 +813,6 @@
         B2_CUDA(ctx, cudaFuncSetAttribute(sixel_palette_kernel<false>, cudaFuncAttributeMaxDynamicSharedMemorySize, 65536));
         B2_CUDA(ctx, cudaFuncSetAttribute(sixel_emit_kernel, cudaFuncAttributeMaxDynamicSharedMemorySize, (int)smem_limit));
         B2_CUDA(ctx, cudaFuncSetAttribute(sixel_emit1b_kernel, cudaFuncAttributeMaxDynamicSharedMemorySize, (227 - 47) * 1024));
-        B2_CUDA(ctx, cudaFuncSetAttribute(sixel_dither_kernel, cudaFuncAttributeMaxDynamicSharedMemorySize, 32768 + DW_MAX * DWARP_SMEM));
         B2_CUDA(ctx, cudaFuncSetAttribute(sixel_palette_kernel<true>, cudaFuncAttributeMaxDynamicSharedMemorySize, 200 * 1024));
         ctx->sixel_attrs_set = true;
     }
@@ -997,7 +826,7 @@
     SixelWork W = S.W;
     const long long npix = S.npix;
     W.hdr += f0; W.ent_a += (long long)f0 * W.ent_cap; W.ent_b += (long long)f0 * W.ent_cap; W.lut += (long long)f0 * 32768;
-    W.index += (long long)f0 * npix; W.boundary += (long long)f0 * W.nb32 * w;
+    W.index += (long long)f0 * npix;
     W.band_bytes += (long long)f0 * W.nbands; W.band_off += (long long)f0 * W.nbands;
     W.scratch += (size_t)f0 * W.nbands * W.band_cap;
     const uint32_t *fb = reinterpret_cast<const uint32_t *>(d_fb) + (long long)f0 * npix;
@@ -1019,17 +848,8 @@
         sixel_map_kernel<<<dim3((unsigned)blocks, n), 256, 0, ctx->stream>>>(fb, npix, W);
         B2_LAUNCH_CHECK(ctx);
     }
-    if (!S.dither_v1) {
-        B2_TRY(launch_sixel_dither(ctx, fb, w, h, n, n_total, W, base + S.o_d2_bnd + sizeof(uint4) * (size_t)f0 * W.nb32 * w,
-                                   base + S.o_d2_prog + sizeof(int) * (size_t)f0 * W.nb32));
-    } else {
-        B2_KERNEL(ctx, "sixel_dither_kernel");
-        const int rounds = (W.nb32 + DW_MAX - 1) / DW_MAX;
-        const int nwarps = (W.nb32 + rounds - 1) / rounds;
-        const size_t dsmem = 32768 + (size_t)nwarps * DWARP_SMEM;
-        sixel_dither_kernel<<<n, nwarps * 32, dsmem, ctx->stream>>>(fb, w, h, nwarps, W);
-        B2_LAUNCH_CHECK(ctx);
-    }
+    B2_TRY(launch_sixel_dither(ctx, fb, w, h, n, n_total, W, base + S.o_d2_bnd + sizeof(uint4) * (size_t)f0 * W.nb32 * w,
+                               base + S.o_d2_prog + sizeof(int) * (size_t)f0 * W.nb32));
     if (S.emit_v1) {
         B2_KERNEL(ctx, "sixel_emit_kernel");
         if (S.emit_mode == 4) sixel_emit1b_kernel<<<dim3(W.nbands, n), ET, S.emit_smem, ctx->stream>>>(S.G, W);
diff --git a/timg_b200/csrc/sixel.cuh b/timg_b200/csrc/sixel.cuh
--- a/timg_b200/csrc/sixel.cuh
+++ b/timg_b200/csrc/sixel.cuh
@@ -16,7 +16,6 @@
     uint32_t *ent_a, *ent_b;
     uint8_t *lut;
     uint8_t *index;
-    uint32_t *boundary;
     uint32_t *band_bytes;
     uint32_t *band_off;
     char *scratch;
diff --git a/timg_b200/csrc/sixel_dither.cu b/timg_b200/csrc/sixel_dither.cu
--- a/timg_b200/csrc/sixel_dither.cu
+++ b/timg_b200/csrc/sixel_dither.cu
@@ -7,19 +7,32 @@
 
 #ifdef CUSIM
 __device__ __forceinline__ uint32_t prmt(uint32_t a, uint32_t b, uint32_t s) { return __byte_perm(a, b, s); }
+template <int N> __device__ __forceinline__ void cp_async(void *dst, const void *src, bool ok) {
+    if (ok) memcpy(dst, src, N); else memset(dst, 0, N);
+}
+__device__ __forceinline__ void cp_async_commit() {}
+__device__ __forceinline__ void cp_async_wait_all() {}
 #else
 __device__ __forceinline__ uint32_t prmt(uint32_t a, uint32_t b, uint32_t s) {
     uint32_t d;
     asm("prmt.b32 %0, %1, %2, %3;" : "=r"(d) : "r"(a), "r"(b), "r"(s));
     return d;
 }
+template <int N> __device__ __forceinline__ void cp_async(void *dst, const void *src, bool ok) {
+    const uint32_t d = (uint32_t)__cvta_generic_to_shared(dst);
+    asm volatile("cp.async.ca.shared.global [%0], [%1], %2, %3;\n" :: "r"(d), "l"(src), "n"(N), "r"(ok ? N : 0) : "memory");
+}
+__device__ __forceinline__ void cp_async_commit() { asm volatile("cp.async.commit_group;\n" ::: "memory"); }
+__device__ __forceinline__ void cp_async_wait_all() { asm volatile("cp.async.wait_group 0;\n" ::: "memory"); }
 #endif
 
 constexpr int D2_WMAX = 24;
 constexpr int D2_CH = 16;
-constexpr int D2_IN_STRIDE = D2_CH + 1;
+constexpr int D2_IN_STRIDE = D2_CH + 2;
 constexpr int D2_OUT_STRIDE = 20;
-constexpr int D2_WARP_SMEM = 2 * 32 * D2_IN_STRIDE * 4 + 32 * D2_OUT_STRIDE + D2_CH * 16;
+constexpr int D2_OFF_TAP = 0, D2_OFF_PAL = 2048, D2_OFF_PROG = 4096, D2_OFF_LUT = 12288, D2_OFF_WARPS = 45056;
+constexpr int D2_WARP_SMEM = 2 * 32 * D2_IN_STRIDE * 4 + 32 * D2_OUT_STRIDE + 2 * D2_CH * 16;
+static_assert(D2_WARP_SMEM % 16 == 0, "per-warp tiles stay 16-byte aligned");
 
 struct TapW { uint32_t r, g, b; };
 
@@ -32,26 +45,33 @@
     return prmt(t.b, 0u, sel);
 }
 __device__ __forceinline__ uint32_t add_clamp(uint32_t v, uint32_t t) { return __viaddmin_s16x2_relu(v, t, 0x00ff00ffu); }
+__device__ __forceinline__ uint32_t cell15(uint32_t vrg, uint32_t vb) { return ((vrg & 0xf8u) << 7) | ((vrg >> 14) & 0x3e0u) | (vb >> 3); }
+__device__ __forceinline__ TapW tap_words(const uint8_t *s_win, uint32_t vrg, uint32_t vb, uint2 np) {
+    const uint32_t erg = (vrg << 2) + np.x, eb = (vb << 2) + np.y;
+    const uint8_t *tap = s_win + D2_OFF_TAP;
+    return {*reinterpret_cast<const uint32_t *>(tap + (erg & 0xffffu)), *reinterpret_cast<const uint32_t *>(tap + (erg >> 16)),
+            *reinterpret_cast<const uint32_t *>(tap + eb)};
+}
 
 struct Dither2Geom { int w, h, nb32, bands_per_cta, nwarps; unsigned spin_ns; };
 
 __global__ void __launch_bounds__(D2_WMAX * 32)
 sixel_dither2_kernel(const uint32_t *__restrict__ fb, Dither2Geom G, SixelWork W, uint4 *__restrict__ bnd_all, int *__restrict__ gprog_all) {
-    extern __shared__ __align__(16) uint8_t s_dyn2[];
-    __shared__ uint2 s_pal2[256];
-    __shared__ uint32_t s_tap[512];
-    __shared__ volatile int s_progress[2048];
+    extern __shared__ __align__(16) uint8_t s_win[];
+    uint32_t *s_tap = reinterpret_cast<uint32_t *>(s_win + D2_OFF_TAP);
+    uint2 *s_pal2 = reinterpret_cast<uint2 *>(s_win + D2_OFF_PAL);
+    volatile int *s_progress = reinterpret_cast<volatile int *>(s_win + D2_OFF_PROG);
+    const uint8_t *s_lut = s_win + D2_OFF_LUT;
     const int f = blockIdx.y, g = blockIdx.x;
     const SixelFrameHdr *hdr = W.hdr + f;
     if (!hdr->diffuse) return;
     const int tid = threadIdx.x, lane = tid & 31, wid = tid >> 5;
     const int nthreads = G.nwarps * 32, w = G.w, h = G.h;
-    uint8_t *s_lut = s_dyn2;
     for (int i = tid; i < 32768 / 16; i += nthreads)
-        reinterpret_cast<uint4 *>(s_lut)[i] = reinterpret_cast<const uint4 *>(W.lut + (long long)f * 32768)[i];
+        reinterpret_cast<uint4 *>(s_win + D2_OFF_LUT)[i] = reinterpret_cast<const uint4 *>(W.lut + (long long)f * 32768)[i];
     for (int i = tid; i < 256; i += nthreads) {
         const uint32_t p = hdr->palette[i];
-        s_pal2[i] = make_uint2((256u - (p & 0xff)) | ((256u - ((p >> 8) & 0xff)) << 16), (256u - ((p >> 16) & 0xff)) | (256u << 16));
+        s_pal2[i] = make_uint2(((256u - (p & 0xff)) | ((256u - ((p >> 8) & 0xff)) << 16)) << 2, (256u - ((p >> 16) & 0xff)) << 2);
     }
     for (int i = tid; i < 512; i += nthreads) {
         const int e = i - 256;
@@ -62,9 +82,10 @@
     const int nlocal = band_hi - band_lo;
     for (int i = tid; i < nlocal; i += nthreads) s_progress[i] = 0;
     __syncthreads();
-    uint32_t *s_in = reinterpret_cast<uint32_t *>(s_dyn2 + 32768 + (size_t)wid * D2_WARP_SMEM);
+    uint32_t *s_in = reinterpret_cast<uint32_t *>(s_win + D2_OFF_WARPS + (size_t)wid * D2_WARP_SMEM);
     uint8_t *s_out = reinterpret_cast<uint8_t *>(s_in + 2 * 32 * D2_IN_STRIDE);
-    uint4 *s_bnd = reinterpret_cast<uint4 *>(s_out + 32 * D2_OUT_STRIDE);
+    uint4 *s_bin = reinterpret_cast<uint4 *>(s_out + 32 * D2_OUT_STRIDE);
+    uint4 *s_bout = s_bin + D2_CH;
     const uint32_t *frame = fb + (long long)f * w * h;
     uint8_t *index = W.index + (long long)f * w * h;
     uint4 *bnd = bnd_all + (long long)f * G.nb32 * w;
@@ -79,114 +100,104 @@
         const int y = band * 32 + lane;
         const bool row_ok = y < h, last_row = (y == h - 1);
         const bool prev_remote = band > 0 && lb == 0;
-        const bool publish_remote = band + 1 < G.nb32 && band + 1 == band_hi;
+        const bool has_below = band + 1 < G.nb32;
+        const bool publish_remote = has_below && band + 1 == band_hi;
         const uint4 *bin = band > 0 ? bnd + (long long)(band - 1) * w : nullptr;
         uint4 *bout = bnd + (long long)band * w;
         TapW own = Z, a0 = Z, a1 = Z, a2 = Z, e_first = Z;
         const int steps = w + 62, nchunks = (steps + D2_CH - 1) / D2_CH;
-        uint32_t pre[16];
-        auto load_chunk = [&](int c) {
+        auto issue_chunk = [&](int c) {
+            uint32_t *t = s_in + (c & 1) * 32 * D2_IN_STRIDE;
             if (even_w) {
 #pragma unroll
                 for (int i = 0; i < 8; ++i) {
                     const int r = 4 * i + qrow, yy = band * 32 + r, x = c * D2_CH - 2 * r + 2 * qcol;
-                    uint2 v = make_uint2(0u, 0u);
-                    if (yy < h && x >= 0 && x < w) v = *reinterpret_cast<const uint2 *>(frame + (long long)yy * w + x);
-                    pre[2 * i] = v.x; pre[2 * i + 1] = v.y;
+                    const bool ok = yy < h && x >= 0 && x < w;
+                    cp_async<8>(t + r * D2_IN_STRIDE + 2 * qcol, ok ? frame + (long long)yy * w + x : frame, ok);
                 }
             } else {
 #pragma unroll
                 for (int i = 0; i < 16; ++i) {
                     const int r = 2 * i + hrow, yy = band * 32 + r, x = c * D2_CH - 2 * r + hcol;
-                    pre[i] = (yy < h && x >= 0 && x < w) ? frame[(long long)yy * w + x] : 0u;
-                }
-            }
+                    const bool ok = yy < h && x >= 0 && x < w;
+                    cp_async<4>(t + r * D2_IN_STRIDE + hcol, ok ? frame + (long long)yy * w + x : frame, ok);
+                }
+            }
+            cp_async_commit();
         };
-        auto store_chunk = [&](int c) {
-            uint32_t *t = s_in + (c & 1) * 32 * D2_IN_STRIDE;
-            if (even_w) {
-#pragma unroll
-                for (int i = 0; i < 8; ++i) {
-                    uint32_t *q = t + (4 * i + qrow) * D2_IN_STRIDE + 2 * qcol;
-                    q[0] = pre[2 * i]; q[1] = pre[2 * i + 1];
-                }
-            } else {
-#pragma unroll
-                for (int i = 0; i < 16; ++i) t[(2 * i + hrow) * D2_IN_STRIDE + hcol] = pre[i];
-            }
-        };
-        load_chunk(0); store_chunk(0);
+        issue_chunk(0);
+        cp_async_wait_all();
         __syncwarp();
         for (int c = 0; c < nchunks; ++c) {
             const int t0 = c * D2_CH;
-            if (c + 1 < nchunks) load_chunk(c + 1);
-            if (band > 0) {
-                const int need = min(w, t0 + D2_CH + 1);
-                if (lane == 0) {
-                    if (prev_remote) { while (gprog[band - 1] < need) __nanosleep(G.spin_ns); __threadfence(); }
-                    else { while (s_progress[lb - 1] < need) __nanosleep(G.spin_ns); __threadfence_block(); }
-                }
+            if (c + 1 < nchunks) issue_chunk(c + 1);
+            {
+                if (band > 0) {
+                    const int need = min(w, t0 + D2_CH + 1);
+                    if (lane == 0) {
+                        if (prev_remote) { while (gprog[band - 1] < need) __nanosleep(G.spin_ns); __threadfence(); }
+                        else { while (s_progress[lb - 1] < need) __nanosleep(G.spin_ns); __threadfence_block(); }
+                    }
+                    __syncwarp();
+                }
+                const int bx = t0 + 1 + lane;
+                if (lane < D2_CH) s_bin[lane] = band > 0 && bx < w ? __ldcg(bin + bx) : make_uint4(0u, 0u, 0u, 0u);
+                if (c == 0 && lane == 0 && band > 0) { const uint4 q = __ldcg(bin); a0.r = q.x; a0.g = q.y; a0.b = q.z; }
                 __syncwarp();
-                const int bx = t0 + 1 + lane;
-                if (lane < D2_CH) s_bnd[lane] = bx < w ? __ldcg(bin + bx) : make_uint4(0u, 0u, 0u, 0u);
-                if (c == 0 && lane == 0) { const uint4 q = __ldcg(bin); a0.r = q.x; a0.g = q.y; a0.b = q.z; }
-                __syncwarp();
-            }
-            const uint32_t *tin = s_in + (c & 1) * 32 * D2_IN_STRIDE + lane * D2_IN_STRIDE;
+            }
+            const uint2 *tin = reinterpret_cast<const uint2 *>(s_in + (c & 1) * 32 * D2_IN_STRIDE + lane * D2_IN_STRIDE);
+            uint8_t *tout = s_out + lane * D2_OUT_STRIDE;
+            auto receive = [&](int j) {
+                const uint4 q = s_bin[j];
+                TapW n;
+                n.r = __shfl_up_sync(0xffffffffu, own.r, 1); n.g = __shfl_up_sync(0xffffffffu, own.g, 1); n.b = __shfl_up_sync(0xffffffffu, own.b, 1);
+                if (lane == 0) { n.r = q.x; n.g = q.y; n.b = q.z; }
+                a2 = a1; a1 = a0; a0 = n;
+            };
             const bool interior = (t0 - 62 >= 1) && (t0 + D2_CH - 1 <= w - 2) && (band * 32 + 31 < h - 1);
             if (interior) {
-#pragma unroll 4
-                for (int j = 0; j < D2_CH; ++j) {
-                    TapW n;
-                    n.r = __shfl_up_sync(0xffffffffu, own.r, 1); n.g = __shfl_up_sync(0xffffffffu, own.g, 1); n.b = __shfl_up_sync(0xffffffffu, own.b, 1);
-                    if (lane == 0) { if (band > 0) { const uint4 q = s_bnd[j]; n.r = q.x; n.g = q.y; n.b = q.z; } else n = Z; }
-                    a2 = a1; a1 = a0; a0 = n;
-                    const uint32_t px = tin[j];
+                auto step = [&](int j, uint32_t px) {
+                    receive(j);
                     uint32_t vrg = prmt(px, 0u, 0x4140u), vb = prmt(px, 0u, 0x4442u);
                     vrg = add_clamp(vrg, tap_rg<3>(a2)); vb = add_clamp(vb, tap_b<3>(a2));
                     vrg = add_clamp(vrg, tap_rg<2>(a1)); vb = add_clamp(vb, tap_b<2>(a1));
                     vrg = add_clamp(vrg, tap_rg<1>(a0)); vb = add_clamp(vb, tap_b<1>(a0));
                     vrg = add_clamp(vrg, tap_rg<0>(own)); vb = add_clamp(vb, tap_b<0>(own));
-                    const uint32_t cell = ((vrg & 0xf8u) << 7) | ((vrg >> 14) & 0x3e0u) | (vb >> 3);
-                    const uint32_t ci = s_lut[cell];
-                    const uint2 np = s_pal2[ci];
-                    const uint32_t erg = vrg + np.x, eb = vb + np.y;
-                    own.r = s_tap[erg & 0x1ffu]; own.g = s_tap[erg >> 16]; own.b = s_tap[eb & 0x1ffu];
-                    s_out[lane * D2_OUT_STRIDE + j] = (uint8_t)ci;
-                    if (lane == 31) __stcg(bout + (t0 + j - 62), make_uint4(own.r, own.g, own.b, 0u));
+                    const uint32_t ci = s_lut[cell15(vrg, vb)];
+                    own = tap_words(s_win, vrg, vb, s_pal2[ci]);
+                    tout[j] = (uint8_t)ci;
+                    if (lane == 31) s_bout[j] = make_uint4(own.r, own.g, own.b, 0u);
+                };
+#pragma unroll
+                for (int j = 0; j < D2_CH; j += 2) {
+                    const uint2 px = tin[j >> 1];
+                    step(j, px.x); step(j + 1, px.y);
                 }
             } else {
-#pragma unroll 2
-                for (int j = 0; j < D2_CH; ++j) {
-                    const int t = t0 + j, x = t - 2 * lane;
-                    TapW n;
-                    n.r = __shfl_up_sync(0xffffffffu, own.r, 1); n.g = __shfl_up_sync(0xffffffffu, own.g, 1); n.b = __shfl_up_sync(0xffffffffu, own.b, 1);
-                    if (lane == 0) { if (band > 0) { const uint4 q = s_bnd[j]; n.r = q.x; n.g = q.y; n.b = q.z; } else n = Z; }
-                    a2 = a1; a1 = a0; a0 = n;
+                auto step = [&](int j, uint32_t px) {
+                    const int x = t0 + j - 2 * lane;
+                    receive(j);
                     uint32_t ci = 0;
                     if (x >= 0 && x < w && row_ok) {
-                        const uint32_t px = tin[j];
                         uint32_t vrg = prmt(px, 0u, 0x4140u), vb = prmt(px, 0u, 0x4442u);
                         vrg = add_clamp(vrg, tap_rg<3>(a2)); vb = add_clamp(vb, tap_b<3>(a2));
                         vrg = add_clamp(vrg, tap_rg<2>(a1)); vb = add_clamp(vb, tap_b<2>(a1));
                         vrg = add_clamp(vrg, tap_rg<1>(a0)); vb = add_clamp(vb, tap_b<1>(a0));
                         if (x == w - 1) { vrg = add_clamp(vrg, tap_rg<1>(e_first)); vb = add_clamp(vb, tap_b<1>(e_first)); }
                         vrg = add_clamp(vrg, tap_rg<0>(own)); vb = add_clamp(vb, tap_b<0>(own));
-                        const uint32_t cell = ((vrg & 0xf8u) << 7) | ((vrg >> 14) & 0x3e0u) | (vb >> 3);
-                        ci = s_lut[cell];
-                        if (x < w - 1 && !last_row) {
-                            const uint2 np = s_pal2[ci];
-                            const uint32_t erg = vrg + np.x, eb = vb + np.y;
-                            own.r = s_tap[erg & 0x1ffu]; own.g = s_tap[erg >> 16]; own.b = s_tap[eb & 0x1ffu];
-                        } else {
-                            own = Z;
-                        }
+                        ci = s_lut[cell15(vrg, vb)];
+                        own = (x < w - 1 && !last_row) ? tap_words(s_win, vrg, vb, s_pal2[ci]) : Z;
                         if (x == 0) e_first = own;
-                        if (lane == 31) __stcg(bout + x, make_uint4(own.r, own.g, own.b, 0u));
                     } else if (x >= w) {
                         own = Z;
                     }
-                    s_out[lane * D2_OUT_STRIDE + j] = (uint8_t)ci;
+                    tout[j] = (uint8_t)ci;
+                    if (lane == 31) s_bout[j] = make_uint4(own.r, own.g, own.b, 0u);
+                };
+#pragma unroll 1
+                for (int j = 0; j < D2_CH; j += 2) {
+                    const uint2 px = tin[j >> 1];
+                    step(j, px.x); step(j + 1, px.y);
                 }
             }
             __syncwarp();
@@ -206,14 +217,19 @@
                 }
             }
             {
+                const int x = t0 - 62 + lane;
+                if (has_below && lane < D2_CH && x >= 0 && x < w) {
+                    __stcg(bout + x, s_bout[lane]);
+                    if (publish_remote) __threadfence(); else __threadfence_block();
+                }
+                __syncwarp();
                 const int done = min(w, t0 + D2_CH - 62);
-                if (lane == 31 && done > 0) {
-                    if (publish_remote) { __threadfence(); gprog[band] = done; }
-                    __threadfence_block();
+                if (lane == 0 && done > 0) {
+                    if (publish_remote) gprog[band] = done;
                     s_progress[lb] = done;
                 }
             }
-            if (c + 1 < nchunks) store_chunk(c + 1);
+            cp_async_wait_all();
             __syncwarp();
         }
     }
@@ -245,8 +261,8 @@
     const int rounds = (G.bands_per_cta + wmax - 1) / wmax;
     G.nwarps = (G.bands_per_cta + rounds - 1) / rounds;
     if (G.bands_per_cta > 2048) return ctx->fail(B200TIMG_EINVAL, "sixel: frame too tall");
-    const size_t smem = 32768 + (size_t)G.nwarps * D2_WARP_SMEM;
-    B2_CUDA(ctx, cudaFuncSetAttribute(sixel_dither2_kernel, cudaFuncAttributeMaxDynamicSharedMemorySize, 32768 + D2_WMAX * D2_WARP_SMEM));
+    const size_t smem = D2_OFF_WARPS + (size_t)G.nwarps * D2_WARP_SMEM;
+    B2_CUDA(ctx, cudaFuncSetAttribute(sixel_dither2_kernel, cudaFuncAttributeMaxDynamicSharedMemorySize, D2_OFF_WARPS + D2_WMAX * D2_WARP_SMEM));
     if (per_frame > 1) B2_CUDA(ctx, cudaMemsetAsync(d_prog, 0, sizeof(int) * (size_t)G.nb32 * n_frames, ctx->stream));
     B2_KERNEL(ctx, "sixel_dither2_kernel");
     sixel_dither2_kernel<<<dim3(per_frame, n_frames), G.nwarps * 32, smem, ctx->stream>>>(fb, G, W, static_cast<uint4 *>(d_bnd), static_cast<int *>(d_prog));
```

After: 71980 (median of 6 runs). 2.4% higher.
